# gonewest818/raytrace-clj

Hardware: AMD Instinct MI355X
Metric: Msamples/sec (nx*ny*ns) (higher is better)
Workload: dtype f64; 1 GPU; C3: 1920x1080x256spp Shirley cover scene n=50 (10001 spheres), depth 50, thin-lens camera, seeded counter RNG; accel=bvh; 8x8 tiles dealt round-robin to 1 GPU(s); nx=1920, ny=1080, ns=256, spheres=10001, depth=50, accel=bvh, accel_ran=bvh, frames_in_flight=1, launch_form=one GPU

## Files before the change

include/rtmi.h:

```cpp
#ifndef RTMI_H
#define RTMI_H

#include <stdint.h>

#ifdef __cplusplus
extern "C" {
#endif

#define RTMI_OK 0
#define RTMI_E_ARG (-1)
#define RTMI_E_DEVICE (-2)
#define RTMI_E_UNSUPPORTED (-3)
#define RTMI_E_NOMEM (-4)
#define RTMI_E_STATE (-5)

enum { RTMI_PRIM_SPHERE = 0, RTMI_PRIM_UVSPHERE = 1, RTMI_PRIM_MOVING = 2,
       RTMI_PRIM_RECT_XY = 3, RTMI_PRIM_RECT_XZ = 4, RTMI_PRIM_RECT_YZ = 5, RTMI_PRIM_TRIANGLE = 6,
       RTMI_PRIM_MEDIUM = 7, RTMI_PRIM_BOUNDARY = 16 };
enum { RTMI_XFORM_TRANSLATE = 0, RTMI_XFORM_ROTATE_Y = 1 };
enum { RTMI_MAT_LAMBERTIAN = 0, RTMI_MAT_METAL = 1, RTMI_MAT_DIELECTRIC = 2, RTMI_MAT_DIFFUSE_LIGHT = 3,
       RTMI_MAT_ISOTROPIC = 4  };
enum { RTMI_TEX_CONSTANT = 0, RTMI_TEX_UVGRADIENT = 1, RTMI_TEX_CHECKER = 2,
       RTMI_TEX_PERLIN_NOISE = 3, RTMI_TEX_PERLIN_TURB = 4, RTMI_TEX_MARBLE = 5, RTMI_TEX_FLIP_U = 6, RTMI_TEX_FLIP_V = 7,
       RTMI_TEX_IMAGE = 8 };
// ... 20 lines not shown
int rtmi_shutdown(rtmi_ctx *ctx);
int rtmi_set_option(rtmi_ctx *ctx, const char *name, int64_t value);
int rtmi_device_info(rtmi_ctx *ctx, int32_t *compute_units, int32_t *lds_bytes_per_cu, int64_t *hbm_bytes, char *arch, int32_t arch_len);

int rtmi_scene_create(rtmi_ctx *ctx,
                      int32_t n_prims, const int32_t *prim_kind, const double *prim_geom, const int32_t *prim_mat,
                      int32_t n_mats, const int32_t *mat_kind, const int32_t *mat_tex, const double *mat_param,
                      int32_t n_tex, const int32_t *tex_kind, const double *tex_param, const int32_t *tex_child,
                      int32_t cam_kind, const double *cam, rtmi_scene **out_scene);
int rtmi_scene_create_ex(rtmi_ctx *ctx,
                         int32_t n_prims, const int32_t *prim_kind, const double *prim_geom, const int32_t *prim_mat,
                         int32_t n_mats, const int32_t *mat_kind, const int32_t *mat_tex, const double *mat_param,
                         int32_t n_tex, const int32_t *tex_kind, const double *tex_param, const int32_t *tex_child,
                         int32_t cam_kind, const double *cam,
                         const int32_t *prim_flip, const int32_t *prim_xform,
                         int32_t n_xforms, const int32_t *xform_kind, const double *xform_param, rtmi_scene **out_scene);
int rtmi_scene_set_perlin(rtmi_scene *scene, const double *vectors, const int32_t *perm);
int rtmi_scene_set_images(rtmi_scene *scene, int32_t n_images, const int32_t *wh, const uint8_t *rgb);
int rtmi_scene_set_media_calls(rtmi_scene *scene, int32_t n_calls, const int32_t *calls);
enum { RTMI_MEDIA_DESCENT = 0, RTMI_MEDIA_HITLIST = 1 };
int rtmi_scene_set_media_mode(rtmi_scene *scene, int32_t mode);
int rtmi_scene_set_media_calls_narrowed(rtmi_scene *scene, int32_t n_calls, const int32_t *calls, const int32_t *narrow_from);
int rtmi_scene_device_bytes(rtmi_scene *scene, int64_t *out_bytes);
int rtmi_scene_destroy(rtmi_scene *scene);

int rtmi_render(rtmi_scene *scene, int32_t nx, int32_t ny, int32_t ns, int32_t depth, uint64_t seed, int32_t precision,
                int32_t x0, int32_t y0, int32_t x1, int32_t y1,
                double *out_linear, uint8_t *out_rgb8, uint64_t *out_counters);

int rtmi_render_device(rtmi_scene *scene, int32_t nx, int32_t ny, int32_t ns, int32_t depth, uint64_t seed, int32_t precision,
                       void *d_out_linear, void *d_out_rgb8, void *d_out_counters, void *stream);

int rtmi_render_tiles_device(rtmi_scene *scene, int32_t nx, int32_t ny, int32_t ns, int32_t depth, uint64_t seed, int32_t precision,
                             int32_t tile_first, int32_t tile_stride,
                             void *d_tiles_linear, void *d_out_counters, void *stream);
int32_t rtmi_local_tiles(int32_t nx, int32_t ny, int32_t tile_first, int32_t tile_stride);

int rtmi_render_progressive(rtmi_scene *scene, int32_t nx, int32_t ny, int32_t s_first, int32_t s_count, int32_t depth, uint64_t seed,
                            int32_t precision, int32_t x0, int32_t y0, int32_t x1, int32_t y1,
                            double *out_linear, uint8_t *out_rgb8, double *out_stderr, uint64_t *out_counters);
int rtmi_render_progressive_device(rtmi_scene *scene, int32_t nx, int32_t ny, int32_t s_first, int32_t s_count, int32_t depth, uint64_t seed,
                                   int32_t precision, void *d_out_linear, void *d_out_rgb8, void *d_out_stderr, void *d_out_counters, void *stream);
int rtmi_progressive_samples(rtmi_ctx *ctx, int32_t *samples);
int rtmi_progressive_release(rtmi_ctx *ctx);

int rtmi_assemble_device(rtmi_ctx *ctx, int32_t nx, int32_t ny, int32_t world, int32_t tiles_per_rank,
                         const void *d_gathered, void *d_out_linear, void *d_out_rgb8, void *stream);

int rtmi_scene_clone(rtmi_scene *scene, rtmi_ctx *ctx, rtmi_scene **out_scene);
int rtmi_render_multi(int32_t n, rtmi_scene *const *scenes, int32_t nx, int32_t ny, int32_t ns, int32_t depth, uint64_t seed,
                      int32_t precision, double *out_linear, uint8_t *out_rgb8, uint64_t *out_counters);
int rtmi_render_multi_device(int32_t n, rtmi_scene *const *scenes, int32_t nx, int32_t ny, int32_t ns, int32_t depth, uint64_t seed,
                             int32_t precision, void *d_out_linear, void *d_out_rgb8, void *d_out_counters);
enum { RTMI_GATHER_NONE = 0,
       RTMI_GATHER_SAME_DEVICE = 1,
       RTMI_GATHER_PEER_COPY = 2,
       RTMI_GATHER_RCCL = 3 };
int rtmi_last_gather_path(rtmi_ctx *ctx0, int32_t *path);
int rtmi_rccl_probe(const char *soname);
int rtmi_stream_idle(rtmi_ctx *ctx, int32_t *idle);
int rtmi_last_passes(rtmi_ctx *ctx, int32_t *passes);
int rtmi_last_accel(rtmi_ctx *ctx, int32_t *accel);
int rtmi_last_gather_ms(rtmi_ctx *ctx0, double *ms);

int rtmi_last_traversal_counters(rtmi_ctx *ctx, uint64_t *out_aabb_tests, uint64_t *out_prim_tests);

int rtmi_last_trace_ms(rtmi_ctx *ctx, double *ms, int32_t *launches);
int rtmi_last_reduce_ms(rtmi_ctx *ctx, double *ms, int32_t *launches);

int rtmi_probe_hit(rtmi_scene *scene, int32_t precision, int32_t n, const double *rays, double t_min, double t_max, double *out);
int rtmi_probe_paths(rtmi_scene *scene, int32_t precision, int32_t n, const double *rays, const uint64_t *keys, uint64_t ctr0,
                     int32_t depth, double *out_rgb, uint64_t *out_nseg, double *log, int32_t max_seg, int32_t *out_nlog);
int rtmi_probe_camera(rtmi_scene *scene, int32_t precision, int32_t n, const double *uv, const uint64_t *keys, double *out);
int rtmi_probe_texture(rtmi_scene *scene, int32_t precision, int32_t tex, int32_t n, const double *uvp, double *out);
int rtmi_probe_scatter(rtmi_scene *scene, int32_t precision, int32_t mat, int32_t n, const double *rays, const double *hits,
                       const uint64_t *keys, double *out);
int rtmi_probe_rng(rtmi_ctx *ctx, int32_t precision, uint64_t key, uint64_t d0, int32_t n, uint64_t *out_bits, double *out_real);
uint64_t rtmi_sample_key(uint64_t seed, uint64_t pixel, uint64_t sample);
int rtmi_probe_arith(rtmi_ctx *ctx, int32_t n, const double *abc, double *out);
#define RTMI_PROBE_MATH_SLOTS 12
int rtmi_probe_math2(rtmi_ctx *ctx, int32_t n, const double *abc, double tmin, double tmax, int32_t n_slots, double *out);
int rtmi_probe_math(rtmi_ctx *ctx, int32_t n, const double *abc, double tmin, double tmax, double *out);

int rtmi_test_build_tree(int32_t n, const double *geom, const double *cam, int32_t threads, uint64_t *out_hash, int32_t *out_info, double *out_ms);
int rtmi_test_half_outward(double x, int32_t up);

#ifdef __cplusplus
}
#endif
#endif
```

raytrace_clj_amd/_ffi.py:

```python
import ctypes as C
import os

import numpy as np

try:
    import torch
except ImportError:
    torch = None

_HERE = os.path.dirname(os.path.abspath(__file__))
LIB_PATH = os.environ.get("RTMI_LIB") or os.path.join(_HERE, "lib", "librtmi.so")

SYMBOLS = [
    "rtmi_last_error", "rtmi_backend_name", "rtmi_version", "rtmi_init", "rtmi_shutdown", "rtmi_set_option",
    "rtmi_device_info", "rtmi_scene_create", "rtmi_scene_create_ex", "rtmi_scene_set_perlin", "rtmi_scene_set_images", "rtmi_scene_set_media_calls", "rtmi_scene_set_media_mode", "rtmi_scene_set_media_calls_narrowed", "rtmi_scene_device_bytes", "rtmi_scene_destroy", "rtmi_render", "rtmi_render_device",
    "rtmi_render_tiles_device", "rtmi_local_tiles", "rtmi_assemble_device", "rtmi_last_trace_ms", "rtmi_last_reduce_ms", "rtmi_probe_hit",
    "rtmi_probe_paths", "rtmi_probe_camera", "rtmi_probe_texture", "rtmi_probe_scatter", "rtmi_probe_rng",
    "rtmi_sample_key", "rtmi_test_half_outward", "rtmi_test_build_tree", "rtmi_probe_arith", "rtmi_probe_math", "rtmi_probe_math2", "rtmi_last_traversal_counters",
    "rtmi_scene_clone", "rtmi_render_multi", "rtmi_render_multi_device", "rtmi_last_gather_ms",
    "rtmi_last_gather_path", "rtmi_rccl_probe", "rtmi_stream_idle", "rtmi_last_passes", "rtmi_last_accel",
    "rtmi_render_progressive", "rtmi_render_progressive_device", "rtmi_progressive_samples", "rtmi_progressive_release",
]

F64, F32 = 0, 1
ACCEL_FLAT, ACCEL_BVH = 0, 1
FLAG_TIMING = 1
GATHER_PATHS = {0: "none", 1: "same-device", 2: "peer-copy", 3: "rccl"}
SEG_REC = 12
TILE = 8


class RtmiError(RuntimeError):
    def __init__(self, code, msg):
        super().__init__("rtmi error %d: %s" % (code, msg))
        self.code = code


_lib = None


def lib():
    global _lib
    if _lib is not None:
        return _lib
    if not os.path.exists(LIB_PATH):
        raise RtmiError(-2, "HIP extension %s is missing; build it with `make -C raytrace_clj_amd/csrc` "
                            "(there is no CPU fallback)" % LIB_PATH)
    L = C.CDLL(LIB_PATH)
    vp, i32, i64, u64, dbl = C.c_void_p, C.c_int32, C.c_int64, C.c_uint64, C.c_double
    L.rtmi_last_error.restype = C.c_char_p
    L.rtmi_backend_name.restype = C.c_char_p
    L.rtmi_version.restype = C.c_int
    L.rtmi_init.argtypes = [C.c_int, C.c_uint32, C.POINTER(vp)]
    L.rtmi_shutdown.argtypes = [vp]
    L.rtmi_set_option.argtypes = [vp, C.c_char_p, i64]
    L.rtmi_device_info.argtypes = [vp, C.POINTER(i32), C.POINTER(i32), C.POINTER(i64), C.c_char_p, i32]
    L.rtmi_scene_create.argtypes = [vp, i32, vp, vp, vp, i32, vp, vp, vp, i32, vp, vp, vp, i32, vp, C.POINTER(vp)]
    L.rtmi_scene_create_ex.argtypes = [vp, i32, vp, vp, vp, i32, vp, vp, vp, i32, vp, vp, vp, i32, vp, vp, vp, i32, vp, vp, C.POINTER(vp)]
    L.rtmi_scene_set_perlin.argtypes = [vp, vp, vp]
    L.rtmi_scene_set_images.argtypes = [vp, i32, vp, vp]
    L.rtmi_scene_set_media_calls.argtypes = [vp, i32, vp]
    L.rtmi_scene_set_media_mode.argtypes = [vp, i32]
    L.rtmi_scene_set_media_calls_narrowed.argtypes = [vp, i32, vp, vp]
    L.rtmi_scene_device_bytes.argtypes = [vp, C.POINTER(C.c_int64)]
    L.rtmi_scene_destroy.argtypes = [vp]
    L.rtmi_render.argtypes = [vp, i32, i32, i32, i32, u64, i32, i32, i32, i32, i32, vp, vp, vp]
    L.rtmi_render_device.argtypes = [vp, i32, i32, i32, i32, u64, i32, vp, vp, vp, vp]
    L.rtmi_render_tiles_device.argtypes = [vp, i32, i32, i32, i32, u64, i32, i32, i32, vp, vp, vp]
    L.rtmi_local_tiles.argtypes = [i32, i32, i32, i32]
    L.rtmi_local_tiles.restype = i32
    L.rtmi_assemble_device.argtypes = [vp, i32, i32, i32, i32, vp, vp, vp, vp]
    L.rtmi_last_trace_ms.argtypes = [vp, C.POINTER(dbl), C.POINTER(i32)]
    L.rtmi_last_reduce_ms.argtypes = [vp, C.POINTER(dbl), C.POINTER(i32)]
    L.rtmi_probe_hit.argtypes = [vp, i32, i32, vp, dbl, dbl, vp]
    L.rtmi_probe_paths.argtypes = [vp, i32, i32, vp, vp, u64, i32, vp, vp, vp, i32, vp]
    L.rtmi_probe_camera.argtypes = [vp, i32, i32, vp, vp, vp]
    L.rtmi_probe_texture.argtypes = [vp, i32, i32, i32, vp, vp]
    L.rtmi_probe_scatter.argtypes = [vp, i32, i32, i32, vp, vp, vp, vp]
    L.rtmi_probe_rng.argtypes = [vp, i32, u64, u64, i32, vp, vp]
    L.rtmi_sample_key.argtypes = [u64, u64, u64]
    L.rtmi_sample_key.restype = u64
    L.rtmi_probe_arith.argtypes = [vp, i32, vp, vp]
    L.rtmi_test_build_tree.argtypes = [i32, vp, vp, i32, vp, vp, vp]
    L.rtmi_test_half_outward.argtypes = [C.c_double, i32]
    L.rtmi_probe_math.argtypes = [vp, i32, vp, C.c_double, C.c_double, vp]
    L.rtmi_probe_math2.argtypes = [vp, i32, vp, C.c_double, C.c_double, i32, vp]
    L.rtmi_last_traversal_counters.argtypes = [vp, C.POINTER(u64), C.POINTER(u64)]
    L.rtmi_scene_clone.argtypes = [vp, vp, C.POINTER(vp)]
    L.rtmi_render_multi.argtypes = [i32, C.POINTER(vp), i32, i32, i32, i32, u64, i32, vp, vp, vp]
    L.rtmi_render_multi_device.argtypes = [i32, C.POINTER(vp), i32, i32, i32, i32, u64, i32, vp, vp, vp]
    L.rtmi_last_gather_ms.argtypes = [vp, C.POINTER(dbl)]
    L.rtmi_last_gather_path.argtypes = [vp, C.POINTER(i32)]
    L.rtmi_rccl_probe.argtypes = [C.c_char_p]
    L.rtmi_stream_idle.argtypes = [vp, C.POINTER(i32)]
    L.rtmi_last_passes.argtypes = [vp, C.POINTER(i32)]
    L.rtmi_last_accel.argtypes = [vp, C.POINTER(i32)]
    L.rtmi_render_progressive.argtypes = [vp, i32, i32, i32, i32, i32, u64, i32, i32, i32, i32, i32, vp, vp, vp, vp]
    L.rtmi_render_progressive_device.argtypes = [vp, i32, i32, i32, i32, i32, u64, i32, vp, vp, vp, vp, vp]
    L.rtmi_progressive_samples.argtypes = [vp, C.POINTER(i32)]
    L.rtmi_progressive_release.argtypes = [vp]
    for name in SYMBOLS:
        fn = getattr(L, name)
        if fn.restype is C.c_int and name not in ("rtmi_version",):
            fn.restype = C.c_int
    _lib = L
    return L


def check(rc):
    if rc != 0:
        raise RtmiError(rc, lib().rtmi_last_error().decode("utf-8", "replace"))


def ptr(a):
    if a is None:
        return None
    if isinstance(a, int):
        return C.c_void_p(a)
    if isinstance(a, np.ndarray):
        return a.ctypes.data_as(C.c_void_p)
    if hasattr(a, "data_ptr"):
        return C.c_void_p(a.data_ptr())
    raise TypeError("cannot take a pointer of %r" % type(a))
```

raytrace_clj_amd/core.py:

```python
import ctypes as C
import sys
import time

import numpy as np

from . import _ffi
from . import camera as cam
from . import flatten as fl
from . import hitable as hitm
from . import shader as shad
from . import texture as texm
from ._ffi import F32, F64, RtmiError, check, ptr

T_MIN = 0.001
T_MAX = 3.4028234663852886e38
DEFAULT_DEPTH = 50
RENDER_SEED = 0x5EED0002

_PRECISION = {"f64": F64, "f32": F32, F64: F64, F32: F32}


class Context:

    def __init__(self, device=0, timing=False):
# ... 138 lines not shown
        return lin, q, err, cnt

    def render_progressive_device(self, nx, ny, s_first, s_count, out_linear=None, out_rgb8=None, out_stderr=None, out_counters=None,
                                  depth=DEFAULT_DEPTH, seed=RENDER_SEED, precision="f64", stream=None):
        check(_ffi.lib().rtmi_render_progressive_device(self.handle, nx, ny, s_first, s_count, depth, seed, _PRECISION[precision],
                                                        ptr(out_linear), ptr(out_rgb8), ptr(out_stderr), ptr(out_counters), ptr(stream)))

    def refine(self, nx, ny, ns, chunk, depth=DEFAULT_DEPTH, seed=RENDER_SEED, precision="f64", region=None):
        if chunk <= 0 or ns <= 0:
            raise ValueError("ns and chunk must be > 0")
        k = 0
        while k < ns:
            n = min(chunk, ns - k)
            lin, q, err, cnt = self.render_progressive(nx, ny, k, n, depth, seed, precision, region)
            k += n
            yield k, lin, q, err, cnt

    def render_tiles_device(self, nx, ny, ns, tile_first, tile_stride, out_tiles, out_counters=None, depth=DEFAULT_DEPTH,
                            seed=RENDER_SEED, precision="f64", stream=None):
        check(_ffi.lib().rtmi_render_tiles_device(self.handle, nx, ny, ns, depth, seed, _PRECISION[precision],
                                                  tile_first, tile_stride, ptr(out_tiles), ptr(out_counters), ptr(stream)))

    def probe_hit(self, rays, t_min=T_MIN, t_max=T_MAX, precision="f64"):
        rays = np.ascontiguousarray(rays, np.float64).reshape(-1, 7)
        out = np.zeros((len(rays), 11), np.float64)
        check(_ffi.lib().rtmi_probe_hit(self.handle, _PRECISION[precision], len(rays), ptr(rays), t_min, t_max, ptr(out)))
        return out

    def probe_paths(self, rays, keys, depth=DEFAULT_DEPTH, ctr0=0, max_seg=0, precision="f64"):
        rays = np.ascontiguousarray(rays, np.float64).reshape(-1, 7)
        keys = np.ascontiguousarray(keys, np.uint64)
        n = len(rays)
        rgb, nseg, nlog = np.zeros((n, 3)), np.zeros(n, np.uint64), np.zeros(n, np.int32)
        log = np.zeros((n, max_seg, _ffi.SEG_REC)) if max_seg else None
        check(_ffi.lib().rtmi_probe_paths(self.handle, _PRECISION[precision], n, ptr(rays), ptr(keys), ctr0, depth,
                                          ptr(rgb), ptr(nseg), ptr(log), max_seg, ptr(nlog)))
        return rgb, nseg, log, nlog

    def probe_camera(self, uv, keys, precision="f64"):
        uv = np.ascontiguousarray(uv, np.float64).reshape(-1, 2)
        keys = np.ascontiguousarray(keys, np.uint64)
        out = np.zeros((len(uv), 8))
        check(_ffi.lib().rtmi_probe_camera(self.handle, _PRECISION[precision], len(uv), ptr(uv), ptr(keys), ptr(out)))
        return out

    def probe_texture(self, tex, uvp, precision="f64"):
        uvp = np.ascontiguousarray(uvp, np.float64).reshape(-1, 5)
        out = np.zeros((len(uvp), 3))
        check(_ffi.lib().rtmi_probe_texture(self.handle, _PRECISION[precision], int(tex), len(uvp), ptr(uvp), ptr(out)))
        return out

    def probe_scatter(self, mat, rays, hits, keys, precision="f64"):
        rays = np.ascontiguousarray(rays, np.float64).reshape(-1, 7)
        hits = np.ascontiguousarray(hits, np.float64).reshape(-1, 8)
        keys = np.ascontiguousarray(keys, np.uint64)
        out = np.zeros((len(rays), 9))
        check(_ffi.lib().rtmi_probe_scatter(self.handle, _PRECISION[precision], int(mat), len(rays), ptr(rays), ptr(hits),
                                            ptr(keys), ptr(out)))
        return out


def probe_rng(key, d0, n, precision="f64", ctx=None):
    ctx = ctx or default_context()
    bits, real = np.zeros(n, np.uint64), np.zeros(n, np.float64)
    check(_ffi.lib().rtmi_probe_rng(ctx.handle, _PRECISION[precision], key, d0, n, ptr(bits), ptr(real)))
    return bits, real


def probe_arith(abc, ctx=None):
    ctx = ctx or default_context()
    abc = np.ascontiguousarray(abc, np.float64).reshape(-1, 3)
    out = np.zeros_like(abc)
    check(_ffi.lib().rtmi_probe_arith(ctx.handle, len(abc), ptr(abc), ptr(out)))
    return out


def probe_math(abc, tmin=0.001, tmax=3.4028234663852886e38, ctx=None):
    ctx = ctx or default_context()
    abc = np.ascontiguousarray(abc, np.float64).reshape(-1, 3)
    slots = 12
    out = np.zeros((len(abc), slots))
    check(_ffi.lib().rtmi_probe_math2(ctx.handle, len(abc), ptr(abc), tmin, tmax, slots, ptr(out)))
    return out


def sample_key(seed, pixel, sample):
    return int(_ffi.lib().rtmi_sample_key(seed, pixel, sample))


_dummy_camera = None


def _one_off(world_items, camera=None):
    global _dummy_camera
    if camera is None:
        if _dummy_camera is None:
            _dummy_camera = cam.PinholeCamera(np.zeros(3), np.zeros(3), np.zeros(3), np.zeros(3))
        camera = _dummy_camera
    return DeviceScene(hitm.Hitlist(list(world_items)), camera)


def _ray7(r):
    return np.concatenate([np.asarray(r["origin"], np.float64), np.asarray(r["direction"], np.float64), [float(r["time"])]])


def hit(obj, r, t_min, t_max):
    items = [obj] if not isinstance(obj, (list, tuple)) else obj
    ds = _one_off(items)
    try:
        o = ds.probe_hit(_ray7(r), float(t_min), float(t_max))[0]
        leaves = []
        fl._leaves(items, leaves, set())
    finally:
        ds.close()
    if o[0] == 0:
        return None
    return {"t": o[2], "p": o[3:6].copy(), "uv": (o[9], o[10]), "normal": o[6:9].copy(), "material": leaves[int(o[1])][0].material}


class _Holder(hitm.Sphere):
    pass


def scatter(material, ray_in, hrec, key=0):
    ds = _one_off([hitm.Sphere(np.zeros(3), 1.0, material)])
    try:
        uv = hrec.get("uv", (0.0, 0.0))
        h = np.concatenate([np.asarray(hrec["p"], np.float64), np.asarray(hrec["normal"], np.float64), [uv[0], uv[1]]])
        o = ds.probe_scatter(0, _ray7(ray_in), h, np.array([key], np.uint64))[0]
    finally:
        ds.close()
    if o[0] == 0:
        return None
    return {"scattered": {"origin": np.asarray(hrec["p"], np.float64), "direction": o[1:4].copy(), "time": o[7]},
            "attenuation": o[4:7].copy()}


def emitted(material, uv, p):
    if isinstance(material, shad.DiffuseLight):
        return sample(material.tex, uv, p)
    return np.zeros(3)


def sample(tex, uv, p):
    ds = _one_off([hitm.Sphere(np.zeros(3), 1.0, shad.Lambertian(tex))])
    try:
        t = int(ds.flat.mat_tex[0])
        return ds.probe_texture(t, np.concatenate([[uv[0], uv[1]], np.asarray(p, np.float64)]))[0]
    finally:
        ds.close()


def get_ray(camera, u, v, key=0):
    ds = _one_off([], camera)
    try:
        o = ds.probe_camera(np.array([u, v], np.float64), np.array([key], np.uint64))[0]
    finally:
        ds.close()
    return {"origin": o[0:3].copy(), "direction": o[3:6].copy(), "time": o[6]}


def render(scene, nx, ny, ns, depth=DEFAULT_DEPTH, seed=RENDER_SEED, precision="f64", ctx=None):
    ds = DeviceScene(scene, ctx=ctx)
    try:
        return ds.render(nx, ny, ns, depth, seed, precision)
    finally:
# ... 125 lines not shown
```

raytrace_clj_amd/csrc/rtmi.hip:

```cpp
#include <hip/hip_runtime.h>
#include <rccl/rccl.h>
#include <dlfcn.h>

#include <algorithm>
#include <atomic>
#include <chrono>
#include <condition_variable>
#include <functional>
#include <thread>
#include <cmath>
#include <cmath>
#include <cstdarg>
#include <cstdio>
#include <cstdlib>
#include <cstring>
#include <array>
#include <map>
#include <mutex>
#include <new>
#include <string>
#include <vector>

#include "rtmi.h"
#include "rtmi_device.h"

using namespace rtmi;

#define RTMI_EXPORT extern "C" __attribute__((visibility("default")))

namespace {

constexpr int kBlock = RTMI_TRACE_BLOCK;
constexpr int kTraceBlock = RTMI_TRACE_BLOCK;
#ifdef RTMI_STAMPS
__device__ unsigned long long g_wg_t[2][4096];
__device__ inline unsigned long long real_now() { unsigned long long t; asm volatile("s_memrealtime %0\n\ts_waitcnt lgkmcnt(0)" : "=s"(t)::"memory"); return t; }
#define RTMI_STAMP_DECL const unsigned long long st_wg0 = real_now(); \
    if (lane == 0) for (int k_ = 0; k_ < 3 * PH_SLOTS + 2; ++k_) g_ph[threadIdx.x >> 6][k_] = 0; \
    ph_stamp(-1); for (int k_ = 0; k_ < 32; ++k_) ph_stamp(PH_CAL);
#define RTMI_STAMP_FLUSH(cnt) if (lane == 0) for (int k_ = 0; k_ < 3 * PH_SLOTS; ++k_) if (g_ph[threadIdx.x >> 6][k_]) atomicAdd(&g_phase[k_], g_ph[threadIdx.x >> 6][k_]); \
    __syncthreads(); if (threadIdx.x == 0 && blockIdx.x < 4096) { g_wg_t[0][blockIdx.x] = st_wg0; g_wg_t[1][blockIdx.x] = real_now(); }
#else
#define RTMI_STAMP_DECL
#define RTMI_STAMP_FLUSH(cnt)
#endif
#ifndef RTMI_MIN_WAVES
#define RTMI_MIN_WAVES 4
#endif
#ifndef RTMI_EXT_MIN_WAVES
#define RTMI_EXT_MIN_WAVES RTMI_MIN_WAVES
#endif

struct TraceParams {
    int nx, ny, depth;
    u64 seed;
    int tiles_x;
    int n_local_tiles;
    const int *tile_ids;
    int s_begin, s_count;
    void *samples;
    u64 *counters;
    int prims_per_tile;
    int n_ptiles;
    unsigned *queue;
    unsigned total_items;
    unsigned qblock;
    int suspend_lanes;
    int rx0, ry0, rx1, ry1;
    u64 *trav;
    int susp_off;
    int stash_off;
};
#ifndef RTMI_QUEUE_BLOCK
#define RTMI_QUEUE_BLOCK 256
#endif
#ifndef RTMI_EXT_NO_STASH
#define RTMI_EXT_NO_STASH 0
#endif
#ifndef RTMI_EXT_LDS_STASH
#define RTMI_EXT_LDS_STASH 1
#endif
#ifndef RTMI_STASH
#define RTMI_STASH 1
#endif
constexpr unsigned kQueueBlock = RTMI_QUEUE_BLOCK;

template <typename R> __device__ inline const R *stat4_of(SceneRef sc);
template <typename R> __device__ inline void stage_prims(SceneRef sc, Prim4<R> *lds, int first, int count) {
    for (int i = threadIdx.x; i < count; i += blockDim.x) {
        const R *g = stat4_of<R>(sc) + (size_t)(first + i) * 4;
        Prim4<R> p;
        p.cx = g[0]; p.cy = g[1]; p.cz = g[2]; p.r2 = g[3];
        lds[i] = p;
    }
}

template <typename R> __device__ inline const R *stat4_of(SceneRef sc);
template <> __device__ inline const double *stat4_of<double>(SceneRef sc) { return sc.stat4_d; }
template <> __device__ inline const float *stat4_of<float>(SceneRef sc) { return sc.stat4_f; }

__device__ inline void scan_cull_dispatch(SceneRef sc, const Path<double> &P, double a, double tmin, double &best_t, int &best_i) {
    scan_all_cull(sc, P, a, tmin, best_t, best_i);
}
__device__ inline void scan_cull_dispatch(SceneRef sc, const Path<float> &P, float a, float tmin, float &best_t, int &best_i) {
    scan_static_pipe<float, false>(ScalarPrims<float>(sc.stat4_f), sc.n_static, 0, P, a, tmin, best_t, best_i);
    if (best_i >= 0) best_i = sc.stat_orig[best_i];
    if (sc.n_moving > 0) {
        int best_orig = best_i >= 0 ? best_i : 0x7fffffff, scan_i = -1;
        scan_moving<float>(sc, P, a, tmin, best_t, scan_i, best_orig);
        if (scan_i >= 0) best_i = best_orig;
    }
}


template <bool SLICED = false, bool COUNT = false, int MSEQ = 0>
__device__ inline void intersect_ext(SceneRef sc, int *stack, bool bvh, Path<double> &P, bool active, double tmin, double tmax, double &best_t, int &best_i,
                                     bool *mid = nullptr, int min_lanes = 0, unsigned *cnt = nullptr, int susp_off = RTMI_BVH_STACK * RTMI_BVH_STRIDE) {
    best_t = tmax; best_i = -1;
    if (!active) return;
    const double a = dot3(P.dx, P.dy, P.dz, P.dx, P.dy, P.dz);
    ExtHit H = {tmax, 0x7fffffff, -1};
    if (MSEQ == 2) {
        MediumChord chord = medium_chord_begin(P);
        ExtHit Hrun = {tmax, 0x7fffffff, -1};
        int cur_lo = -1, scanned_to = 0;
        for (int k = 0; k < sc.n_media; ++k) {
            const int m = sc.media_idx[k], lo = sc.media_lo[k];
            if (lo >= m) { ext_medium_test(sc, m, P, tmin, tmax, H, chord, COUNT ? cnt : nullptr); continue; }
            if (lo != cur_lo) { Hrun.t = tmax; Hrun.F = 0x7fffffff; Hrun.W = -1; cur_lo = lo; scanned_to = lo; }
            if (m > scanned_to) scan_all_cull_ext(sc, P, a, tmin, Hrun, scanned_to, m);
            double tm = 0.0;
            if (ext_medium_test(sc, m, P, tmin, Hrun.any() ? Hrun.t : tmax, Hrun, chord, COUNT ? cnt : nullptr, &tm)) ext_update(H, tm, m, true);
            scanned_to = m + 1;
        }
        if (bvh) scan_bvh_ext<false, COUNT>(sc, stack, P, a, tmin, H, nullptr, false, 0, cnt);
        else if (sc.small_scan) scan_small_ext(sc, P, tmin, H);
        else scan_all_cull_ext(sc, P, a, tmin, H);
        best_i = ext_winner(H);
        if (best_i >= 0) best_t = H.t;
        return;
    }
    if (MSEQ == 1) {
        int prev = 0;
        MediumChord chord = medium_chord_begin(P);
        for (int k = 0; k <= sc.n_media; ++k) {
            const int m = k < sc.n_media ? sc.media_idx[k] : sc.n_all;
            if (m > prev) {
                if (bvh) scan_bvh_ext<false, COUNT>(sc, stack, P, a, tmin, H, nullptr, false, 0, cnt, prev, m);
                else if (sc.small_scan) scan_small_ext(sc, P, tmin, H, prev, m);
                else scan_all_cull_ext(sc, P, a, tmin, H, prev, m);
            }
            if (k < sc.n_media) ext_medium_test(sc, m, P, tmin, H.any() ? H.t : tmax, H, chord, COUNT ? cnt : nullptr);
            prev = m + 1;
        }
        best_i = ext_winner(H);
        if (best_i >= 0) best_t = H.t;
        return;
    }
    if (!(SLICED && bvh && *mid)) {
        MediumChord chord = medium_chord_begin(P);
        for (int k = 0; k < sc.n_media; ++k) ext_medium_test(sc, sc.media_idx[k], P, tmin, tmax, H, chord, COUNT ? cnt : nullptr, nullptr, k);
        RTMI_PH(PH_MEDIA)
    }
    if (bvh) {
        if (SLICED) {
            const bool done = scan_bvh_ext<true, COUNT>(sc, stack, P, a, tmin, H, stack + susp_off, *mid, min_lanes, cnt);
            *mid = !done;
            if (!done) return;
        } else scan_bvh_ext<false, COUNT>(sc, stack, P, a, tmin, H, nullptr, false, 0, cnt);
    } else if (sc.small_scan) scan_small_ext(sc, P, tmin, H);
    else scan_all_cull_ext(sc, P, a, tmin, H);
    RTMI_PH(PH_BVH_POST)
    best_i = ext_winner(H);
    if (best_i >= 0) best_t = H.t;
}
template <bool SLICED = false, bool COUNT = false, int MSEQ = 0>
__device__ inline void intersect_ext(SceneRef, int *, bool, Path<float> &, bool, float, float tmax, float &best_t, int &best_i, bool * = nullptr, int = 0, unsigned * = nullptr, int = 0) { best_t = tmax; best_i = -1; }

template <typename R, bool MULTI, int VARIANT, bool EXT = false, bool COUNT = false, bool SLICED = false, int MSEQ = 0, bool NOGRID = false>
__device__ inline void intersect_world(SceneRef sc, Prim4<R> *lds, int prims_per_tile, int n_ptiles, Path<R> &P,
                                       bool active, R tmin, R tmax, R &best_t, int &best_i, unsigned *cnt = nullptr, bool *mid = nullptr, int min_lanes = 0,
                                       int susp_off = RTMI_BVH_STACK * RTMI_BVH_STRIDE) {
    if (EXT) { intersect_ext<SLICED, COUNT, MSEQ>(sc, reinterpret_cast<int *>(lds), VARIANT == SCAN_BVH, P, active, tmin, tmax, best_t, best_i, mid, min_lanes, cnt, susp_off); return; }
    best_t = tmax;
    best_i = -1;
    const R a = dot3(P.dx, P.dy, P.dz, P.dx, P.dy, P.dz);
    if (VARIANT == SCAN_BVH) {
        int *stack = reinterpret_cast<int *>(lds);
        if (active) {
            if (SLICED) {
                const bool done = scan_bvh<R, COUNT, true>(sc, stack, P, a, tmin, best_t, best_i, [&]() { scan_cull_dispatch(sc, P, a, tmin, best_t, best_i); }, cnt,
                                                           stack + susp_off, *mid, min_lanes);
                *mid = !done;
            } else scan_bvh<R, COUNT, false, !NOGRID>(sc, stack, P, a, tmin, best_t, best_i, [&]() { scan_cull_dispatch(sc, P, a, tmin, best_t, best_i); }, cnt);
        }
        return;
    }
    if (VARIANT == SCAN_SGPR_CULL) {
        if (active) scan_cull_dispatch(sc, P, a, tmin, best_t, best_i);
        return;
    }
    if (VARIANT == SCAN_SGPR) {
        if (active) scan_static_pipe<R, false>(ScalarPrims<R>(stat4_of<R>(sc)), sc.n_static, 0, P, a, tmin, best_t, best_i);
    } else if (!MULTI) {
        if (active) {
            if (VARIANT == SCAN_LDS_PIPE) scan_static_pipe<R, true>(LdsPrims<R>{lds}, sc.n_static, 0, P, a, tmin, best_t, best_i);
            else scan_static<R>(lds, sc.n_static, 0, P, a, tmin, best_t, best_i);
        }
    } else {
        for (int tile = 0; tile < n_ptiles; ++tile) {
            const int first = tile * prims_per_tile;
            const int count = min(prims_per_tile, sc.n_static - first);
            __syncthreads();
            stage_prims<R>(sc, lds, first, count);
            __syncthreads();
            if (active) {
                if (VARIANT == SCAN_LDS_PIPE) scan_static_pipe<R, true>(LdsPrims<R>{lds}, count, first, P, a, tmin, best_t, best_i);
                else scan_static<R>(lds, count, first, P, a, tmin, best_t, best_i);
            }
        }
    }
    if (active) {
        if (best_i >= 0) best_i = sc.stat_orig[best_i];
        if (sc.n_moving > 0) {
            int best_orig = best_i >= 0 ? best_i : 0x7fffffff, scan_i = -1;
            scan_moving<R>(sc, P, a, tmin, best_t, scan_i, best_orig);
            if (scan_i >= 0) best_i = best_orig;
        }
    }
}

template <typename R> __device__ inline void start_sample(SceneRef sc, const TraceParams &tp, int i, int j, int s, Path<R> &P) {
    seed_stream(P, sample_key(tp.seed, (u64)j * (u64)tp.nx + (u64)i, (u64)s), 0u);
    const R u = ((R)(float)i + next_uniform(P)) / (R)tp.nx;
    const R v = ((R)(float)j + next_uniform(P)) / (R)tp.ny;
    get_ray<R>(sc, u, v, P);
    P.ar = P.ag = P.ab = R(1);
    P.depth = tp.depth;
}

template <typename R, bool MULTI, int VARIANT, bool EXT = false, bool COUNT = false, bool SLICE = true, int MSEQ = 0, bool LST = false>
__global__ void __launch_bounds__(kTraceBlock, EXT ? ((MSEQ != 0 || COUNT) ? 3 : RTMI_EXT_MIN_WAVES) : RTMI_MIN_WAVES) trace_kernel(ScenePtr scp, TraceParams tp) {
    SceneRef sc = *scp;
    extern __shared__ __attribute__((aligned(16))) char smem[];
    Prim4<R> *lds = reinterpret_cast<Prim4<R> *>(smem);
    const int lane = threadIdx.x & 63;
    if (!MULTI && VARIANT < SCAN_SGPR) stage_prims<R>(sc, lds, 0, sc.n_static);
    __syncthreads();

    const unsigned total_items = tp.total_items;
    unsigned w_cur = 0, w_end = 0;
    Path<R> P;
    P.ox = P.oy = P.oz = P.dx = P.dy = P.dz = P.time = R(0);
    P.ar = P.ag = P.ab = R(0);
    seed_stream(P, 0ull, 0u); P.depth = 0;
    bool alive = false;
    bool exhausted = (total_items == 0);
    unsigned out_item = 0;
    constexpr bool LSTASH = (EXT && RTMI_STASH && RTMI_EXT_LDS_STASH && !RTMI_EXT_NO_STASH) || LST;
    constexpr bool STASH = RTMI_STASH && !(EXT && RTMI_EXT_NO_STASH) && !LSTASH;
    int *const lst = reinterpret_cast<int *>(smem) + tp.stash_off + (threadIdx.x & ~63);
    R st_ox = R(0), st_oy = R(0), st_oz = R(0), st_dx = R(0), st_dy = R(0), st_dz = R(0), st_time = R(0);
    u64 st_rs = 0;
    unsigned st_item = 0xffffffffu;
    unsigned s_head = 64u;
    unsigned nrays = 0;
    unsigned ntrav[2] = {0u, 0u};
    const R tmin = R(0.001), tmax = Real<R>::tmax();
    constexpr bool SLICED = SLICE && VARIANT == SCAN_BVH && !MULTI;
    bool mid = false;

    RTMI_STAMP_DECL
    for (;;) {
        RTMI_PH(PH_LOOP)
        if (LSTASH) {
        for (;;) {
            const u64 dead = __ballot(!alive);
            if (dead == 0) break;
            if (s_head == 64u) {
                if (exhausted) break;
                if (w_cur == w_end) {
                    unsigned base = 0;
                    if (lane == 0) base = atomicAdd(tp.queue, tp.qblock);
                    base = __builtin_amdgcn_readfirstlane(base);
                    if (base >= total_items) { exhausted = true; break; }
                    w_cur = base;
                    w_end = min(base + tp.qblock, total_items);
                }
                const unsigned m = w_cur + (unsigned)lane;
                w_cur += 64u;
                const unsigned chunk = m >> 6;
                const int l = (int)(m & 63u);
                const int tile_local = (int)(chunk / (unsigned)tp.s_count);
                const int s = tp.s_begin + (int)(chunk - (unsigned)tile_local * (unsigned)tp.s_count);
                const int gtile = tp.tile_ids[tile_local];
                const int x = (gtile % tp.tiles_x) * RTMI_TILE + (l & 7);
                const int y = (gtile / tp.tiles_x) * RTMI_TILE + (l >> 3);
                unsigned item = 0xffffffffu;
                if (x >= tp.rx0 && x < tp.rx1 && y >= tp.ry0 && y < tp.ry1) {
                    Path<R> Q;
                    start_sample<R>(sc, tp, x, tp.ny - 1 - y, s, Q);
                    int w0, w1;
                    best_to_words<R>(Q.dx, w0, w1); lst[lane] = w0; lst[kTraceBlock + lane] = w1;
                    best_to_words<R>(Q.dy, w0, w1); lst[2 * kTraceBlock + lane] = w0; lst[3 * kTraceBlock + lane] = w1;
                    best_to_words<R>(Q.dz, w0, w1); lst[4 * kTraceBlock + lane] = w0; lst[5 * kTraceBlock + lane] = w1;
                    best_to_words<R>(Q.time, w0, w1); lst[6 * kTraceBlock + lane] = w0; lst[7 * kTraceBlock + lane] = w1;
                    lst[8 * kTraceBlock + lane] = (int)(unsigned)Q.rs; lst[9 * kTraceBlock + lane] = (int)(unsigned)(Q.rs >> 32);
                    if (!sc.cam_fixed_origin) {
                        best_to_words<R>(Q.ox, w0, w1); lst[11 * kTraceBlock + lane] = w0; lst[12 * kTraceBlock + lane] = w1;
                        best_to_words<R>(Q.oy, w0, w1); lst[13 * kTraceBlock + lane] = w0; lst[14 * kTraceBlock + lane] = w1;
                        best_to_words<R>(Q.oz, w0, w1); lst[15 * kTraceBlock + lane] = w0; lst[16 * kTraceBlock + lane] = w1;
                    }
                    item = m;
                    RTMI_PH(PH_REFILL_GEN)
                }
                lst[10 * kTraceBlock + lane] = (int)item;
                s_head = 0u;
            }
// ... 713 lines not shown
    fprintf(stderr, "[phases] one stamp = %.0f ticks; stamps took %.1f %% of the %.4g wave-ticks of this (diagnostic) launch and are subtracted below\n", per_stamp, 100 * (raw - tot) / raw, raw);
    fprintf(stderr, "[phases] %-36s %8s %8s %10s %10s %12s\n", "phase", "ticks %", "lanes", "masked %", "useful %", "stamps");
    for (int k = 0; k < PH_N; ++k) {
        if (!h[k] || k == PH_CAL) continue;
        const double t = tk[k], l = lk[k];
        fprintf(stderr, "[phases] %-36s %8.2f %8.1f %10.2f %10.2f %12llu\n", names[k], 100 * t / tot, t > 0 ? l / t : 0.0, 100 * (64 * t - l) / (64 * tot), 100 * l / (64 * tot), h[2 * PH_SLOTS + k]);
    }
    fprintf(stderr, "[phases] %-36s %8.2f %8.1f %10.2f %10.2f   (%.4g wave-ticks)\n", "total", 100.0, totl / tot, 100 * (64 * tot - totl) / (64 * tot), 100 * totl / (64 * tot), tot);
    return RTMI_OK;
}
#endif

template <typename R>
int render_passes(rtmi_scene *s, int nx, int ny, int s_first, int s_end, int depth, uint64_t seed, int first, int stride, const int *rg, void *d_tiles_linear,
                  void *d_counters, hipStream_t st, ProgFrame *prog) {
    rtmi_ctx *c = s->ctx;
    int n_local = 0;
    const int whole[4] = {0, 0, nx, ny};
    if (!rg) rg = whole;
    int rc = ensure_tile_ids(c, nx, ny, first, stride, rg, st, &n_local);
    if (rc) return rc;
    c->last_stream = st;
    if (c->fail_next_render) { c->fail_next_render = 0; return fail(RTMI_E_DEVICE, "render failed (injected by the test hook test_fail_next_render)"); }
    if (prog) {
        prog->k = 0;
        const size_t elems = (size_t)std::max(n_local, 1) * 192;
        if (s_first == 0) {
            rc = prog->sums.ensure(elems * sizeof(R));
            if (!rc) rc = prog->mean.ensure(elems * sizeof(double));
            if (!rc) rc = prog->m2.ensure(elems * sizeof(double));
            if (!rc) rc = prog->counters.ensure(2 * sizeof(u64));
            if (rc) return rc;
            HIP_TRY(hipMemsetAsync(prog->counters.p, 0, 2 * sizeof(u64), st));
        } else if (prog->sums.bytes < elems * sizeof(R) || prog->m2.bytes < elems * sizeof(double)) {
            return fail(RTMI_E_STATE, "progressive frame buffers do not match the frame");
        }
        d_counters = prog->counters.p;
    }
    rc = c->counters.ensure(8 * sizeof(u64));
    if (rc) return rc;
    if (d_counters && !prog) HIP_TRY(hipMemsetAsync(d_counters, 0, 2 * sizeof(u64), st));
    HIP_TRY(hipMemsetAsync(reinterpret_cast<u64 *>(c->counters.p) + 3, 0, 2 * sizeof(u64), st));
    if (n_local == 0) return RTMI_OK;
    u64 *cnt = d_counters ? reinterpret_cast<u64 *>(d_counters) : reinterpret_cast<u64 *>(c->counters.p);
    unsigned *queue = reinterpret_cast<unsigned *>(reinterpret_cast<u64 *>(c->counters.p) + 2);

    const int ns = s_end - s_first;
    const size_t per_sample = (size_t)n_local * 64 * 3 * sizeof(R);
    int s_per_pass = (int)std::max<int64_t>(1, std::min<int64_t>(ns, c->workspace_bytes / (int64_t)per_sample));
    while (s_per_pass > 1 && (long long)n_local * s_per_pass * 64 >= 0xf0000000ll) s_per_pass /= 2;
    if ((long long)n_local * s_per_pass * 64 >= 0xf0000000ll) return fail(RTMI_E_ARG, "frame too large for one pass: %d tiles per rank", n_local);
    if (per_sample * (size_t)s_per_pass > c->samples.bytes) {
        constexpr double kFreeShare = 0.8;
        size_t free_b = 0, total_b = 0;
        if (hipMemGetInfo(&free_b, &total_b) == hipSuccess) {
            const double avail = kFreeShare * (double)free_b + (double)c->samples.bytes;
            const int fit = (int)std::max<double>(1.0, std::min<double>((double)s_per_pass, avail / (double)per_sample));
            s_per_pass = std::min(s_per_pass, fit);
        }
        for (;;) {
            if (c->fail_allocs > 0) { c->fail_allocs--; c->samples.release(); rc = fail(RTMI_E_NOMEM, "hipMalloc(%zu bytes) failed (injected by the test hook)", per_sample * (size_t)s_per_pass); }
            else rc = c->samples.ensure(per_sample * (size_t)s_per_pass);
            if (!rc) break;
            (void)hipGetLastError();
            if (s_per_pass == 1) return rc;
            s_per_pass = (s_per_pass + 1) / 2;
        }
    }
    c->last_passes = (ns + s_per_pass - 1) / s_per_pass;
    if (!prog && s_per_pass < ns) {
        rc = c->accum.ensure((size_t)n_local * 64 * 3 * sizeof(R));
        if (rc) return rc;
    }
    int ppt, nptiles;
    size_t lds_bytes;
    lds_plan(c, s->dev.n_static, sizeof(R), &ppt, &nptiles, &lds_bytes);
    const TracePlan plan = choose_trace_kernel<R>(s, c, read_launch_knobs(), nptiles > 1, lds_bytes);
    c->last_accel = plan.accel;

    for (int s_begin = s_first; s_begin < s_end; s_begin += s_per_pass) {
        const int s_count = std::min(s_per_pass, s_end - s_begin);
        TraceParams tp;
        tp.nx = nx; tp.ny = ny; tp.depth = depth; tp.seed = seed; tp.tiles_x = tiles_x_of(nx);
        tp.n_local_tiles = n_local; tp.tile_ids = reinterpret_cast<const int *>(c->tile_ids.p);
        tp.s_begin = s_begin; tp.s_count = s_count; tp.samples = c->samples.p; tp.counters = cnt;
        tp.prims_per_tile = (c->scan_variant >= SCAN_SGPR || s->dev.has_ext) ? 0 : ppt; tp.n_ptiles = nptiles;
        hipEvent_t e0 = nullptr, e1 = nullptr;
        if ((c->flags & RTMI_FLAG_TIMING) && c->events_used < 8192) {
            rc = next_event_pair(c, &e0, &e1);
            if (rc) return rc;
            HIP_TRY(hipEventRecord(e0, st));
        }
        tp.queue = queue; tp.total_items = (unsigned)((long long)n_local * s_count * 64);
        {
            const long long per_wave = (long long)tp.total_items / std::max(1, c->cus * 16);
            unsigned qb = s->dev.has_ext ? 192u : kQueueBlock;
            while (qb < 1024u && per_wave >= (long long)qb * 128) qb *= 2;
            if (const char *e = std::getenv("RTMI_QUEUE_BLOCK_RT")) qb = std::max(64, std::atoi(e) / 64 * 64);
            tp.qblock = qb;
        }
        tp.rx0 = std::max(rg[0], 0); tp.ry0 = std::max(rg[1], 0); tp.rx1 = std::min(rg[2], nx); tp.ry1 = std::min(rg[3], ny);
        tp.trav = reinterpret_cast<u64 *>(c->counters.p) + 3;
        tp.suspend_lanes = plan.suspend_lanes; tp.susp_off = plan.lds.susp_off; tp.stash_off = plan.lds.stash_off;
        HIP_TRY(hipMemsetAsync(queue, 0, sizeof(unsigned), st));
        int resident = 0;
        {
            const std::pair<const void *, size_t> key(reinterpret_cast<const void *>(plan.kern), plan.lds.bytes);
            auto it = c->occupancy.find(key);
            if (it == c->occupancy.end()) {
                HIP_TRY(hipOccupancyMaxActiveBlocksPerMultiprocessor(&resident, plan.kern, kTraceBlock, plan.lds.bytes));
                c->occupancy.emplace(key, resident);
            } else resident = it->second;
        }
        const int grid_trace = std::max(1, c->cus * std::max(1, std::min(c->blocks_per_cu * (256 / kTraceBlock), resident)));
        if (c->last_grid != grid_trace && std::getenv("RTMI_DEBUG"))
            fprintf(stderr, "[rtmi] trace launch: %d workgroups of %d threads (%d resident per CU by the occupancy query, cap %d), %zu B LDS each\n",
                    grid_trace, kTraceBlock, resident, c->blocks_per_cu * (256 / kTraceBlock), plan.lds.bytes);
        c->last_grid = grid_trace;
        hipLaunchKernelGGL(plan.kern, dim3(grid_trace), dim3(kTraceBlock), plan.lds.bytes, st, s->d_dev, tp);
        HIP_TRY(hipGetLastError());
        if (e1) HIP_TRY(hipEventRecord(e1, st));
        const long long npx = (long long)n_local * 64;
        if (prog)
            hipLaunchKernelGGL((progressive_fold_kernel<R>), dim3((unsigned)((npx + kBlock - 1) / kBlock)), dim3(kBlock), 0, st,
                               reinterpret_cast<const R *>(c->samples.p), reinterpret_cast<R *>(prog->sums.p), reinterpret_cast<double *>(prog->mean.p),
                               reinterpret_cast<double *>(prog->m2.p), reinterpret_cast<const int *>(c->tile_ids.p), tiles_x_of(nx), n_local,
                               s_begin, s_count, cnt, (u64)c->tile_valid_pixels, tp.rx0, tp.ry0, tp.rx1, tp.ry1);
        else
            hipLaunchKernelGGL((reduce_kernel<R>), dim3((unsigned)((npx + kBlock - 1) / kBlock)), dim3(kBlock), 0, st,
                               reinterpret_cast<const R *>(c->samples.p), reinterpret_cast<R *>(c->accum.p),
                               reinterpret_cast<double *>(d_tiles_linear), reinterpret_cast<const int *>(c->tile_ids.p), tiles_x_of(nx), nx, ny,
                               n_local, s_begin, s_count, ns, d_counters ? cnt : nullptr, (u64)c->tile_valid_pixels, tp.rx0, tp.ry0, tp.rx1, tp.ry1);
        HIP_TRY(hipGetLastError());
        if (e1) {
            const size_t k = (size_t)c->events_used - 1;
            while (c->events_r.size() <= k) { hipEvent_t e; HIP_TRY(hipEventCreate(&e)); c->events_r.push_back(e); }
            HIP_TRY(hipEventRecord(c->events_r[k], st));
        }
    }
#ifdef RTMI_STAMPS
    rc = report_phase_stamps(c, st);
#endif
    if (!rc && prog) prog->k = s_end;
    return rc;
}

template <typename R>
int render_tiles_impl(rtmi_scene *s, int nx, int ny, int ns, int depth, uint64_t seed, int first, int stride, const int *rg, void *d_tiles_linear,
                      void *d_counters, hipStream_t st) {
    return render_passes<R>(s, nx, ny, 0, ns, depth, seed, first, stride, rg, d_tiles_linear, d_counters, st, nullptr);
}

int check_render_args(rtmi_scene *s, int nx, int ny, int ns, int depth, int precision) {
    if (!scene_ok(s)) return fail(RTMI_E_STATE, "invalid scene handle");
    if (nx <= 0 || ny <= 0 || ns <= 0 || depth < 0) return fail(RTMI_E_ARG, "nx, ny, ns must be > 0 and depth >= 0 (got %d %d %d %d)", nx, ny, ns, depth);
    if ((long long)nx * ny > (1ll << 30)) return fail(RTMI_E_ARG, "frame too large");
    if (precision != RTMI_F64 && precision != RTMI_F32) return fail(RTMI_E_ARG, "precision must be RTMI_F64 or RTMI_F32");
    if (precision == RTMI_F32 && s->dev.has_ext) return fail(RTMI_E_UNSUPPORTED, "rectangles / triangles / instances / procedural textures are rendered by the FP64 kernels only");
    if (s->uses_perlin && !s->have_perlin) return fail(RTMI_E_STATE, "the scene holds a Perlin texture: call rtmi_scene_set_perlin first");
    if (s->max_image >= s->dev.n_images) return fail(RTMI_E_STATE, "the scene holds an ImageMap with index %d: call rtmi_scene_set_images first", s->max_image);
    return RTMI_OK;
}

}

RTMI_EXPORT int rtmi_test_build_tree(int32_t n, const double *geom, const double *cam, int32_t threads, uint64_t *out_hash, int32_t *out_info, double *out_ms) {
    if (n <= 0 || !geom || !cam || !out_hash || !out_info || !out_ms) return fail(RTMI_E_ARG, "bad arguments");
    const BuildKnobs knobs = read_build_knobs();
    std::vector<int> kind((size_t)n, RTMI_PRIM_SPHERE);
    std::vector<BvhBox> wbox((size_t)n);
    std::vector<char> bounded((size_t)n, 0), box_first((size_t)n, 0);
    for (int i = 0; i < n; ++i) {
        const double g[9] = {geom[4 * (size_t)i], geom[4 * (size_t)i + 1], geom[4 * (size_t)i + 2], geom[4 * (size_t)i + 3], 0, 0, 0, 0, 1};
        bounded[(size_t)i] = prim_world_box(RTMI_PRIM_SPHERE, g, nullptr, nullptr, 0, 0, 0.0, 1.0, wbox[(size_t)i]);
    }
    DevScene d{};
    std::vector<int> grid_cells;
    int depth = 0;
    g_build_single.store(threads == 1 ? 1 : 0);
    const double t0 = now_ms();
    const std::vector<float> nodes = build_bvh(d, n, kind.data(), wbox, bounded, cam, true, grid_cells, box_first, knobs, &depth);
    *out_ms = now_ms() - t0;
    g_build_single.store(0);
    uint64_t h = 1469598103934665603ull;
    auto mix = [&](const void *p, size_t bytes) { const unsigned char *q = (const unsigned char *)p; for (size_t k = 0; k < bytes; ++k) { h ^= q[k]; h *= 1099511628211ull; } };
    mix(nodes.data(), nodes.size() * sizeof(float));
    mix(grid_cells.data(), grid_cells.size() * sizeof(int));
    mix(&d.bvh_root, sizeof(int)); mix(&d.grid_tall, sizeof(int)); mix(&d.bvh_node16, sizeof(int));
    *out_hash = h;
    out_info[0] = (int32_t)(nodes.size() / (d.bvh_node16 ? 8 : 16)); out_info[1] = depth; out_info[2] = d.grid_n; out_info[3] = d.n_big;
    return RTMI_OK;
}
RTMI_EXPORT int rtmi_test_half_outward(double x, int32_t up) { return (int)half_outward((float)x, up != 0); }
RTMI_EXPORT const char *rtmi_last_error(void) { return g_err.c_str(); }
RTMI_EXPORT const char *rtmi_backend_name(void) { return "hip-gfx950"; }
RTMI_EXPORT int rtmi_version(void) { return 205; }
RTMI_EXPORT uint64_t rtmi_sample_key(uint64_t seed, uint64_t pixel, uint64_t sample) { return sample_key(seed, pixel, sample); }

RTMI_EXPORT int rtmi_init(int device, uint32_t flags, rtmi_ctx **out_ctx) {
    if (!out_ctx) return fail(RTMI_E_ARG, "out_ctx is NULL");
    *out_ctx = nullptr;
    int ndev = 0;
    if (hipGetDeviceCount(&ndev) != hipSuccess || ndev <= 0) return fail(RTMI_E_DEVICE, "no HIP device visible (this library has no CPU fallback)");
    if (device < 0 || device >= ndev) return fail(RTMI_E_ARG, "device %d out of range (0..%d)", device, ndev - 1);
    HIP_TRY(hipSetDevice(device));
    hipDeviceProp_t prop;
    HIP_TRY(hipGetDeviceProperties(&prop, device));
    if (std::strncmp(prop.gcnArchName, "gfx950", 6) != 0)
        return fail(RTMI_E_DEVICE, "device %d is %s; this library carries gfx950 (MI355X) code objects only", device, prop.gcnArchName);
    rtmi_ctx *c = new (std::nothrow) rtmi_ctx();
    if (!c) return fail(RTMI_E_NOMEM, "out of host memory");
    c->device = device;
    c->flags = flags;
    c->cus = prop.multiProcessorCount;
    c->lds_per_cu = (int)prop.maxSharedMemoryPerMultiProcessor;
    c->hbm = prop.totalGlobalMem;
    c->arch = prop.gcnArchName;
    if (const char *e = std::getenv("RTMI_BLOCKS_PER_CU")) c->blocks_per_cu = std::max(1, std::atoi(e));
    if (const char *e = std::getenv("RTMI_SCAN_VARIANT")) c->scan_variant = std::min(3, std::max(0, std::atoi(e)));
    if (const char *e = std::getenv("RTMI_LDS_TILE_BYTES")) c->max_lds_bytes = std::min(64 * 1024 - 64, std::max(1024, std::atoi(e)));
    if (hipStreamCreateWithFlags(&c->stream, hipStreamNonBlocking) != hipSuccess) { delete c; return fail(RTMI_E_DEVICE, "hipStreamCreate failed"); }
    *out_ctx = c;
    return RTMI_OK;
}

RTMI_EXPORT int rtmi_shutdown(rtmi_ctx *c) {
    if (!ctx_ok(c)) return fail(RTMI_E_STATE, "invalid context handle");
    (void)hipSetDevice(c->device);
    (void)hipStreamSynchronize(c->stream);
#ifdef RTMI_HIST
    { unsigned long long h[200]; if (hipMemcpyFromSymbol(h, HIP_SYMBOL(rtmi::g_hist), sizeof h) == hipSuccess) { for (int k = 0; k < 3; ++k) { fprintf(stderr, "HIST%d", k); for (int i = 0; i <= 64; ++i) fprintf(stderr, " %llu", h[64 * k + i]); fprintf(stderr, "\n"); } } }
#endif
    c->samples.release(); c->accum.release(); c->tiles.release(); c->tile_ids.release(); c->counters.release(); c->scratch_lin.release(); c->multi.release();
    c->prog.release();
    for (hipEvent_t e : {c->ev_done, c->ev_g0, c->ev_g1}) if (e) (void)hipEventDestroy(e);
    if (c->ev_consumed) { (void)hipSetDevice(c->ev_consumed_device); (void)hipEventDestroy(c->ev_consumed); (void)hipSetDevice(c->device); }
    for (auto &e : c->events) { (void)hipEventDestroy(e.first); (void)hipEventDestroy(e.second); }
    for (hipEvent_t e : c->events_r) (void)hipEventDestroy(e);
    (void)hipStreamDestroy(c->stream);
    c->magic = 0;
    delete c;
    return RTMI_OK;
}

RTMI_EXPORT int rtmi_set_option(rtmi_ctx *c, const char *name, int64_t value) {
    if (!ctx_ok(c)) return fail(RTMI_E_STATE, "invalid context handle");
    if (!name) return fail(RTMI_E_ARG, "name is NULL");
    if (!std::strcmp(name, "blocks_per_cu")) { if (value < 1 || value > 64) return fail(RTMI_E_ARG, "blocks_per_cu must be 1..64"); c->blocks_per_cu = (int)value; return RTMI_OK; }
    if (!std::strcmp(name, "workspace_bytes")) { if (value < (1 << 20)) return fail(RTMI_E_ARG, "workspace_bytes must be >= 1 MiB"); c->workspace_bytes = value; return RTMI_OK; }
    if (!std::strcmp(name, "lds_tile_bytes")) { if (value < 1024 || value > 64 * 1024 - 64) return fail(RTMI_E_ARG, "lds_tile_bytes out of range"); c->max_lds_bytes = (int)value; return RTMI_OK; }
    if (!std::strcmp(name, "timing")) { if (value) c->flags |= RTMI_FLAG_TIMING; else c->flags &= ~RTMI_FLAG_TIMING; return RTMI_OK; }
    if (!std::strcmp(name, "scan_variant")) { if (value < 0 || value > 3) return fail(RTMI_E_ARG, "scan_variant must be 0..3"); c->scan_variant = (int)value; return RTMI_OK; }
    if (!std::strcmp(name, "count_traversal")) { c->count_traversal = value ? 1 : 0; return RTMI_OK; }
    if (!std::strcmp(name, "test_fail_next_render")) { c->fail_next_render = value ? 1 : 0; return RTMI_OK; }
    if (!std::strcmp(name, "test_fail_allocs")) { c->fail_allocs = (int)std::max<int64_t>(0, std::min<int64_t>(value, 64)); return RTMI_OK; }
    if (!std::strcmp(name, "flat_below")) { if (value < 0 || value > (1 << 20)) return fail(RTMI_E_ARG, "flat_below must be 0..2^20"); c->flat_below = (int)value; return RTMI_OK; }
    if (!std::strcmp(name, "suspend_lanes")) { if (value < 0 || value > 64) return fail(RTMI_E_ARG, "suspend_lanes must be 0..64"); c->suspend_lanes = (int)value; c->suspend_lanes_set = true; return RTMI_OK; }
    if (!std::strcmp(name, "accel")) {
        if (value == RTMI_ACCEL_FLAT || value == RTMI_ACCEL_BVH) { c->accel = (int)value; return RTMI_OK; }
        return fail(RTMI_E_UNSUPPORTED, "accel %lld is not available in this build", (long long)value);
    }
    return fail(RTMI_E_ARG, "unknown option '%s'", name);
}

RTMI_EXPORT int rtmi_device_info(rtmi_ctx *c, int32_t *cus, int32_t *lds, int64_t *hbm, char *arch, int32_t arch_len) {
    if (!ctx_ok(c)) return fail(RTMI_E_STATE, "invalid context handle");
    if (cus) *cus = c->cus;
    if (lds) *lds = c->lds_per_cu;
    if (hbm) *hbm = (int64_t)c->hbm;
    if (arch && arch_len > 0) { std::strncpy(arch, c->arch.c_str(), (size_t)arch_len - 1); arch[arch_len - 1] = 0; }
    return RTMI_OK;
}

RTMI_EXPORT int rtmi_scene_create(rtmi_ctx *c, int32_t n_prims, const int32_t *prim_kind, const double *prim_geom, const int32_t *prim_mat,
                                  int32_t n_mats, const int32_t *mat_kind, const int32_t *mat_tex, const double *mat_param,
                                  int32_t n_tex, const int32_t *tex_kind, const double *tex_param, const int32_t *tex_child,
                                  int32_t cam_kind, const double *cam, rtmi_scene **out_scene) {
    return rtmi_scene_create_ex(c, n_prims, prim_kind, prim_geom, prim_mat, n_mats, mat_kind, mat_tex, mat_param, n_tex, tex_kind, tex_param, tex_child,
                                cam_kind, cam, nullptr, nullptr, 0, nullptr, nullptr, out_scene);
// ... 886 lines not shown
    else hipLaunchKernelGGL((probe_camera_kernel<float>), dim3(grid), dim3(kBlock), 0, c->stream, s->d_dev, n, d_uv, d_keys, d_out);
    PROBE_EPILOGUE()
    HIP_TRY(hipMemcpy(out, d_out, (size_t)n * 8 * sizeof(double), hipMemcpyDeviceToHost));
    return RTMI_OK;
}

RTMI_EXPORT int rtmi_probe_texture(rtmi_scene *s, int32_t precision, int32_t tex, int32_t n, const double *uvp, double *out) {
    PROBE_PROLOGUE(s)
    if (!uvp || !out) return fail(RTMI_E_ARG, "NULL array");
    if (tex < 0 || tex >= s->n_tex) return fail(RTMI_E_ARG, "texture index %d out of range", tex);
    double *d_in = (double *)tmp.up(uvp, (size_t)n * 5 * sizeof(double));
    double *d_out = (double *)tmp.alloc((size_t)n * 3 * sizeof(double));
    if (!d_in || !d_out) return fail(RTMI_E_NOMEM, "probe buffers");
    if (s->dev.has_ext) {
        if (precision != RTMI_F64) return fail(RTMI_E_UNSUPPORTED, "procedural / image textures are FP64 only");
        hipLaunchKernelGGL((probe_texture_kernel<double, true>), dim3(grid), dim3(kBlock), 0, c->stream, s->d_dev, tex, n, d_in, d_out);
    } else if (precision == RTMI_F64) hipLaunchKernelGGL((probe_texture_kernel<double>), dim3(grid), dim3(kBlock), 0, c->stream, s->d_dev, tex, n, d_in, d_out);
    else hipLaunchKernelGGL((probe_texture_kernel<float>), dim3(grid), dim3(kBlock), 0, c->stream, s->d_dev, tex, n, d_in, d_out);
    PROBE_EPILOGUE()
    HIP_TRY(hipMemcpy(out, d_out, (size_t)n * 3 * sizeof(double), hipMemcpyDeviceToHost));
    return RTMI_OK;
}

RTMI_EXPORT int rtmi_probe_scatter(rtmi_scene *s, int32_t precision, int32_t mat, int32_t n, const double *rays, const double *hits,
                                   const uint64_t *keys, double *out) {
    PROBE_PROLOGUE(s)
    if (!rays || !hits || !keys || !out) return fail(RTMI_E_ARG, "NULL array");
    if (mat < 0 || mat >= s->n_mats) return fail(RTMI_E_ARG, "material index %d out of range", mat);
    double *d_rays = (double *)tmp.up(rays, (size_t)n * 7 * sizeof(double));
    double *d_hits = (double *)tmp.up(hits, (size_t)n * 8 * sizeof(double));
    u64 *d_keys = (u64 *)tmp.up(keys, (size_t)n * sizeof(u64));
    double *d_out = (double *)tmp.alloc((size_t)n * 9 * sizeof(double));
    if (!d_rays || !d_hits || !d_keys || !d_out) return fail(RTMI_E_NOMEM, "probe buffers");
    if (s->dev.has_ext) {
        if (precision != RTMI_F64) return fail(RTMI_E_UNSUPPORTED, "procedural / image textures are FP64 only");
        hipLaunchKernelGGL((probe_scatter_kernel<double, true>), dim3(grid), dim3(kBlock), 0, c->stream, s->d_dev, mat, n, d_rays, d_hits, d_keys, d_out);
    } else if (precision == RTMI_F64) hipLaunchKernelGGL((probe_scatter_kernel<double>), dim3(grid), dim3(kBlock), 0, c->stream, s->d_dev, mat, n, d_rays, d_hits, d_keys, d_out);
    else hipLaunchKernelGGL((probe_scatter_kernel<float>), dim3(grid), dim3(kBlock), 0, c->stream, s->d_dev, mat, n, d_rays, d_hits, d_keys, d_out);
    PROBE_EPILOGUE()
    HIP_TRY(hipMemcpy(out, d_out, (size_t)n * 9 * sizeof(double), hipMemcpyDeviceToHost));
    return RTMI_OK;
}

RTMI_EXPORT int rtmi_probe_rng(rtmi_ctx *c, int32_t precision, uint64_t key, uint64_t d0, int32_t n, uint64_t *out_bits, double *out_real) {
    if (!ctx_ok(c)) return fail(RTMI_E_STATE, "invalid context handle");
    if (precision != RTMI_F64 && precision != RTMI_F32) return fail(RTMI_E_ARG, "bad precision");
    if (n <= 0 || !out_bits || !out_real) return fail(RTMI_E_ARG, "bad arguments");
    HIP_TRY(hipSetDevice(c->device));
    Tmp tmp;
    u64 *d_bits = (u64 *)tmp.alloc((size_t)n * sizeof(u64));
    double *d_real = (double *)tmp.alloc((size_t)n * sizeof(double));
    if (!d_bits || !d_real) return fail(RTMI_E_NOMEM, "probe buffers");
    const unsigned grid = (unsigned)((n + kBlock - 1) / kBlock);
    if (precision == RTMI_F64) hipLaunchKernelGGL((probe_rng_kernel<double>), dim3(grid), dim3(kBlock), 0, c->stream, (u64)key, (u64)d0, n, d_bits, d_real);
    else hipLaunchKernelGGL((probe_rng_kernel<float>), dim3(grid), dim3(kBlock), 0, c->stream, (u64)key, (u64)d0, n, d_bits, d_real);
    PROBE_EPILOGUE()
    HIP_TRY(hipMemcpy(out_bits, d_bits, (size_t)n * sizeof(u64), hipMemcpyDeviceToHost));
    HIP_TRY(hipMemcpy(out_real, d_real, (size_t)n * sizeof(double), hipMemcpyDeviceToHost));
    return RTMI_OK;
}

__global__ void probe_math_kernel(int n, const double *abc, double tmin, double tmax, int n_slots, double *out) {
    const int k = blockIdx.x * blockDim.x + threadIdx.x;
    if (k >= n) return;
    const double a = abc[3 * k], b = abc[3 * k + 1], c = abc[3 * k + 2];
    double o[RTMI_PROBE_MATH_SLOTS];
    o[0] = rt_sqrt(a);
    const TrigTable K = trig_table();
    o[1] = rt_atan2(a, b, K);
    o[2] = rt_asin(a, K);
    Real<double>::sphere_uv(a, b, c, &o[3], &o[4]);
    const Quot<double> q = make_quot<double>(b, tmin, tmax);
    o[5] = q(a);
    o[6] = div_const(a, K[29], K[27]);
    o[7] = (double)q.fast;
    o[8] = (double)float_above(c);
    o[9] = rt_log_unit(a);
    const bool fast = rcp_in_range(b) && tmin >= 0x1p-300 && tmax <= 0x1p200;
    o[10] = div_by(a, refined_rcp(b), fast);
    o[11] = (double)fast;
    for (int j = 0; j < n_slots; ++j) out[(size_t)k * n_slots + j] = o[j];
}

RTMI_EXPORT int rtmi_probe_arith(rtmi_ctx *c, int32_t n, const double *abc, double *out) {
    if (!ctx_ok(c)) return fail(RTMI_E_STATE, "invalid context handle");
    if (n <= 0 || !abc || !out) return fail(RTMI_E_ARG, "bad arguments");
    HIP_TRY(hipSetDevice(c->device));
    Tmp tmp;
    double *d_in = (double *)tmp.up(abc, (size_t)n * 3 * sizeof(double));
    double *d_out = (double *)tmp.alloc((size_t)n * 3 * sizeof(double));
    if (!d_in || !d_out) return fail(RTMI_E_NOMEM, "probe buffers");
    const unsigned grid = (unsigned)((n + kBlock - 1) / kBlock);
    hipLaunchKernelGGL(probe_arith_kernel, dim3(grid), dim3(kBlock), 0, c->stream, n, d_in, d_out);
    PROBE_EPILOGUE()
    HIP_TRY(hipMemcpy(out, d_out, (size_t)n * 3 * sizeof(double), hipMemcpyDeviceToHost));
    return RTMI_OK;
}

RTMI_EXPORT int rtmi_probe_math2(rtmi_ctx *c, int32_t n, const double *abc, double tmin, double tmax, int32_t n_slots, double *out) {
    if (!ctx_ok(c)) return fail(RTMI_E_STATE, "invalid context handle");
    if (n <= 0 || !abc || !out) return fail(RTMI_E_ARG, "bad arguments");
    if (n_slots < 1 || n_slots > RTMI_PROBE_MATH_SLOTS) return fail(RTMI_E_ARG, "n_slots must be 1..%d", RTMI_PROBE_MATH_SLOTS);
    HIP_TRY(hipSetDevice(c->device));
    Tmp tmp;
    double *d_in = (double *)tmp.up(abc, (size_t)n * 3 * sizeof(double));
    double *d_out = (double *)tmp.alloc((size_t)n * (size_t)n_slots * sizeof(double));
    if (!d_in || !d_out) return fail(RTMI_E_NOMEM, "probe buffers");
    const unsigned grid = (unsigned)((n + kBlock - 1) / kBlock);
    hipLaunchKernelGGL(probe_math_kernel, dim3(grid), dim3(kBlock), 0, c->stream, n, d_in, tmin, tmax, (int)n_slots, d_out);
    PROBE_EPILOGUE()
    HIP_TRY(hipMemcpy(out, d_out, (size_t)n * (size_t)n_slots * sizeof(double), hipMemcpyDeviceToHost));
    return RTMI_OK;
}
RTMI_EXPORT int rtmi_probe_math(rtmi_ctx *c, int32_t n, const double *abc, double tmin, double tmax, double *out) {
    return rtmi_probe_math2(c, n, abc, tmin, tmax, 8, out);
}
```

raytrace_clj_amd/csrc/rtmi_device.h:

```cpp
#pragma once
#include <hip/hip_runtime.h>
#include <stdint.h>

#include "rtmi.h"

namespace rtmi {

typedef unsigned long long u64;

struct DevScene {
    int n_static;
    int n_moving;
    const double *stat_geom;
    const double *stat4_d;
    const float *stat4_f;
    int n_all;
    const float *cull20;
    const double *exact12;
    double cull_t_lo, cull_t_hi;
    const float *bvh_nodes;
    int bvh_root;
    int n_big;
    int big_idx[16];
    int bvh_node16;
// ... 131 lines not shown
__device__ inline double rt_atan2(double y, double x, TrigTable K) {
    double c_hi = K[11], c_lo = K[12], h_hi = K[13], h_lo = K[14], p_hi = K[15], p_lo = K[16];
    asm volatile("" : "+s"(c_hi), "+s"(c_lo), "+s"(h_hi), "+s"(h_lo), "+s"(p_hi), "+s"(p_lo));
    const double ax = ::fabs(x), ay = ::fabs(y);
    const bool swap = ay > ax;
    const double a = swap ? ax : ay, b = swap ? ay : ax;
    const bool far = a > 0.4375 * b;
    const bool zero = b == 0.0;
    double num = far ? ::fma(-0.75, b, a) : a, den = far ? ::fma(0.75, a, b) : b;
    den = zero ? 1.0 : den;
    const double xr = num / den, z = xr * xr, w = z * z;
    const double s1 = z * fma_s(w, fma_s(w, fma_s(w, fma_s(w, ::fma(w, K[10], K[8]), K[6]), K[4]), K[2]), K[0]);
    const double s2 = w * fma_s(w, fma_s(w, fma_s(w, ::fma(w, K[9], K[7]), K[5]), K[3]), K[1]);
    const double hi = far ? c_hi : 0.0, lo = far ? c_lo : 0.0;
    double r = hi - (::fma(xr, s1 + s2, -lo) - xr);
    const double rs = h_hi - (r - h_lo);
    r = swap ? rs : r;
    const bool neg = (x < 0.0) | (zero & (bool)__builtin_signbit(x));
    const double rn = p_hi - (r - p_lo);
    r = neg ? rn : r;
    return ::copysign(r, y);
}
__device__ inline double rt_asin(double x, TrigTable K) {
    const double ax = ::fabs(x);
    const bool small = ax < 0.5;
    const double t = small ? x * x : ::fma(ax, -0.5, 0.5);
    const double p = t * fma_s(t, fma_s(t, fma_s(t, fma_s(t, ::fma(t, K[22], K[21]), K[20]), K[19]), K[18]), K[17]);
    const double q = ::fma(t, fma_s(t, fma_s(t, ::fma(t, K[26], K[25]), K[24]), K[23]), 1.0);
    const double r = p / q, s = rt_sqrt(t);
    const double big = K[13] - ::fma(2.0, ::fma(s, r, s), -K[14]);
    return ::copysign(small ? ::fma(ax, r, ax) : big, x);
}
__device__ inline double rt_log_unit(double x) {
    const double ln2_hi = 6.93147180369123816490e-01, ln2_lo = 1.90821492927058770002e-10;
    const double Lg1 = 6.666666666666735130e-01, Lg2 = 3.999999999940941908e-01, Lg3 = 2.857142874366239149e-01, Lg4 = 2.222219843214978396e-01,
                 Lg5 = 1.818357216161805012e-01, Lg6 = 1.531383769920937332e-01, Lg7 = 1.479819860511658591e-01;
    int hx = __double2hiint(x);
    const unsigned lx = (unsigned)__double2loint(x);
    if (!(x > 0.0) || hx >= 0x7ff00000) return x == 0.0 ? -__builtin_inf() : ::log(x);
    if (hx < 0x00100000) return ::log(x);
    int k = (hx >> 20) - 1023;
    hx &= 0x000fffff;
    const int i = (hx + 0x95f64) & 0x100000;
    const double m = __hiloint2double(hx | (i ^ 0x3ff00000), (int)lx);
    k += i >> 20;
    const double f = m - 1.0, dk = (double)k;
    const double s = f / (2.0 + f);
    const double z = s * s, w = z * z;
    const double t1 = w * ::fma(w, ::fma(w, Lg6, Lg4), Lg2);
    const double t2 = z * ::fma(w, ::fma(w, ::fma(w, Lg7, Lg5), Lg3), Lg1);
    const double R = t2 + t1, hfsq = 0.5 * f * f;
    return ::fma(dk, ln2_hi, -((hfsq - ::fma(s, hfsq + R, dk * ln2_lo)) - f));
}

__device__ inline double div_const(double x, double c, double rc) {
    const double q = x * rc;
    return ::fma(::fma(-c, q, x), rc, q);
}

template <typename R> struct Quot {
    R a;
    __device__ inline R operator()(R n) const { return n / a; }
};
template <> struct Quot<double> {
    double a, r;
    bool fast;
    __device__ inline double operator()(double n) const {
        if (__builtin_expect(!fast, 0)) return n / a;
        const double q = n * r;
        return ::fma(::fma(-a, q, n), r, q);
    }
};
template <typename R> __device__ inline Quot<R> make_quot(R a, R, R) { return Quot<R>{a}; }
template <> __device__ inline Quot<double> make_quot<double>(double a, double tmin, double tmax) {
    Quot<double> q;
    q.a = a;
    const unsigned hi = (unsigned)__double2hiint(a);
    q.fast = (hi - (823u << 20) < (400u << 20)) && tmin >= 0x1p-300 && tmax <= 0x1p200;
    double r = __builtin_amdgcn_rcp(a);
    r = ::fma(r, ::fma(-a, r, 1.0), r);
    q.r = ::fma(r, ::fma(-a, r, 1.0), r);
    return q;
}
template <typename R> __device__ inline R quot(R n, R a) { return n / a; }
template <typename R> __device__ inline R quot(R n, const Quot<R> &a) { return a(n); }
template <typename R> __device__ inline R coef(R a) { return a; }
template <typename R> __device__ inline R coef(const Quot<R> &a) { return a.a; }

#ifdef RTMI_HIST
__device__ unsigned long long g_hist[200];
#endif
template <typename R> struct Real;
template <> struct Real<double> {
    __device__ static inline double k53(u64 z) { const u64 k = z >> 11; return ::fma((double)(unsigned)(k >> 32), 4294967296.0, (double)(unsigned)k); }
#ifndef RTMI_RNG_BITS
#define RTMI_RNG_BITS 1
#endif
#if RTMI_RNG_BITS
    __device__ static inline double from_bits(u64 z, unsigned expo, unsigned sub_b1, unsigned sub_b0) {
        const unsigned hi = (unsigned)(z >> 32), lo = (unsigned)z;
        const double m = __hiloint2double((int)(expo | ((hi >> 11) & 0x000fffffu)), (int)__builtin_amdgcn_alignbit(hi, lo, 11));
        return m - __hiloint2double((int)hi < 0 ? (int)sub_b1 : (int)sub_b0, 0);
    }
    __device__ static inline double uniform(u64 z) { return from_bits(z, 0x3fe00000u, 0u, 0x3fe00000u); }
    __device__ static inline double symmetric(u64 z) { return from_bits(z, 0x3ff00000u, 0x3ff00000u, 0x40000000u); }
#else
    __device__ static inline double uniform(u64 z) { return k53(z) * (1.0 / 9007199254740992.0); }
    __device__ static inline double symmetric(u64 z) { return ::fma(k53(z), 1.0 / 4503599627370496.0, -1.0); }
#endif
    __device__ static inline double tmax() { return 3.4028234663852886e38; }
    __device__ static inline double pi() { return 3.141592653589793; }
    __device__ static inline double sqrt_(double x) { return rt_sqrt(x); }
    __device__ static inline double sqrt_lib(double x) { return ::sqrt(x); }
    __device__ static inline double sin_(double x) { return ::sin(x); }
    __device__ static inline void sphere_uv(double nx, double ny, double nz, double *u, double *v) { *u = sphere_u(nx, nz); *v = sphere_v(ny); }
    __device__ static inline double sphere_u(double nx, double nz) { const TrigTable K = trig_table(); return 1.0 - div_const(rt_atan2(nz, nx, K) + K[30], K[29], K[27]); }
    __device__ static inline double sphere_v(double ny) { const TrigTable K = trig_table(); return div_const(rt_asin(ny, K) + K[13], K[30], K[28]); }
    __device__ static inline double pow_(double x, double y) { return ::pow(x, y); }
};
template <> struct Real<float> {
    __device__ static inline float uniform(u64 z) { return (float)(unsigned)(z >> 40) * (1.0f / 16777216.0f); }
    __device__ static inline float symmetric(u64 z) { return 2.0f * uniform(z) - 1.0f; }
    __device__ static inline float tmax() { return 3.4028234663852886e38f; }
    __device__ static inline float pi() { return 3.141592653589793f; }
    __device__ static inline float sqrt_(float x) { return ::sqrtf(x); }
    __device__ static inline float sqrt_lib(float x) { return ::sqrtf(x); }
    __device__ static inline float sin_(float x) { return ::sinf(x); }
    __device__ static inline void sphere_uv(float nx, float ny, float nz, float *u, float *v) { *u = sphere_u(nx, nz); *v = sphere_v(ny); }
    __device__ static inline float sphere_u(float nx, float nz) { return 1.0f - (::atan2f(nz, nx) + pi()) / (2.0f * pi()); }
    __device__ static inline float sphere_v(float ny) { return (::asinf(ny) + pi() / 2.0f) / pi(); }
    __device__ static inline float pow_(float x, float y) { return ::powf(x, y); }
};

__device__ inline double pow5(double x) {
    const double h2 = x * x, l2 = ::fma(x, x, -h2);
    const double h4 = h2 * h2, l4 = ::fma(h2, h2, -h4) + 2.0 * (h2 * l2);
    const double h5 = h4 * x, l5 = ::fma(h4, x, -h5) + l4 * x;
    return h5 + l5;
}
__device__ inline float pow5(float x) { const double d = (double)x, d2 = d * d; return (float)(d2 * d2 * d); }

template <typename R> struct Path {
    R ox, oy, oz, dx, dy, dz, time;
    R ar, ag, ab;
    u64 key;
    u64 rs;
    unsigned ctr;
    int depth;
};
template <typename R> __device__ inline void seed_stream(Path<R> &P, u64 key, unsigned ctr0) { P.key = key; P.ctr = ctr0; P.rs = key + RTMI_GOLD * (u64)ctr0; }

template <typename R> __device__ inline R next_uniform(Path<R> &P) {
    P.rs += RTMI_GOLD;
    P.ctr++;
    return Real<R>::uniform(mix64(P.rs));
}

template <typename R> __device__ inline R next_symmetric(Path<R> &P) {
    P.rs += RTMI_GOLD;
    P.ctr++;
    return Real<R>::symmetric(mix64(P.rs));
}

template <typename R> __device__ inline R dot3(R ax, R ay, R az, R bx, R by, R bz) { return (ax * bx + ay * by) + az * bz; }

template <typename R> __device__ inline void rand_in_unit_sphere(Path<R> &P, R &x, R &y, R &z) {
// ... 205 lines not shown
        if (kind == RTMI_TEX_UVGRADIENT) {
            const R omu = R(1.0) - u, omv = R(1.0) - v;
            const R a0 = (R)tp[3] * omu + (R)tp[0] * u, a1 = (R)tp[4] * omu + (R)tp[1] * u, a2 = (R)tp[5] * omu + (R)tp[2] * u;
            const R b0 = (R)tp[9] * omu + (R)tp[6] * u, b1 = (R)tp[10] * omu + (R)tp[7] * u, b2 = (R)tp[11] * omu + (R)tp[8] * u;
            r = b0 * omv + a0 * v; g = b1 * omv + a1 * v; b = b2 * omv + a2 * v;
            return;
        }
        if (kind == RTMI_TEX_CHECKER) {
            const R scale = (R)tp[0];
            const int sx = sin_sign<R>(scale * px), sy = sin_sign<R>(scale * py), sz = sin_sign<R>(scale * pz);
            t = (sx * sy * sz < 0) ? sc.tex_child[2 * t] : sc.tex_child[2 * t + 1];
            continue;
        }
        if (F4) {
            if (kind == RTMI_TEX_PERLIN_NOISE) {
                const R s = (R)tp[0];
                r = g = b = R(0.5) * (perlin_noise<R>(sc, s * px, s * py, s * pz) + R(1.0));
                return;
            }
            if (kind == RTMI_TEX_PERLIN_TURB) {
                const R s = (R)tp[0];
                r = g = b = R(0.5) * (perlin_turbulence<R>(sc, s * px, s * py, s * pz, (int)tp[1]) + R(1.0));
                return;
            }
            if (kind == RTMI_TEX_MARBLE) {
                r = g = b = R(0.5) * (Real<R>::sin_((R)tp[0] * pz + R(10.0) * perlin_turbulence<R>(sc, px, py, pz, (int)tp[1])) + R(1.0));
                return;
            }
            if (kind == RTMI_TEX_FLIP_U) { u = R(1.0) - u; t = sc.tex_child[2 * t]; continue; }
            if (kind == RTMI_TEX_FLIP_V) { v = R(1.0) - v; t = sc.tex_child[2 * t]; continue; }
            if (kind == RTMI_TEX_IMAGE) {
                const int im = (int)tp[0];
                const int w = sc.image_wh[2 * im], h = sc.image_wh[2 * im + 1];
                int i = (int)(u * (R)w), j = (int)(v * (R)h);
                i = i < 0 ? 0 : (i >= w ? w - 1 : i); j = j < 0 ? 0 : (j >= h ? h - 1 : j);
                const unsigned char *q = sc.image_rgb + sc.image_off[im] + ((size_t)j * w + i) * 3;
                r = (R)q[0] / R(255.0); g = (R)q[1] / R(255.0); b = (R)q[2] / R(255.0);
                return;
            }
        }
        return;
    }
}

template <typename R> struct alignas(16) Prim4 { R cx, cy, cz, r2; };

enum { SCAN_LDS_LITERAL = 0, SCAN_LDS_PIPE = 1, SCAN_SGPR = 2, SCAN_SGPR_CULL = 3, SCAN_BVH = 4 };

template <typename R>
__device__ inline void scan_static(const Prim4<R> *__restrict__ lds, int n, int idx_base, const Path<R> &P, R a, R tmin, R &best_t, int &best_i) {
    const R a2 = R(2.0) * a, a4 = R(4.0) * a;
#pragma unroll 2
    for (int i = 0; i < n; ++i) {
        const Prim4<R> s = lds[i];
        const R ocx = P.ox - s.cx, ocy = P.oy - s.cy, ocz = P.oz - s.cz;
        const R b = R(2.0) * dot3(ocx, ocy, ocz, P.dx, P.dy, P.dz);
        const R c = dot3(ocx, ocy, ocz, ocx, ocy, ocz) - s.r2;
        const R disc = b * b - a4 * c;
        if (disc >= R(0)) {
            const R sq = Real<R>::sqrt_lib(disc);
            R t = (-b - sq) / a2;
            bool ok = (t > tmin) && (t < best_t);
            if (!ok) {
                t = (-b + sq) / a2;
                ok = (t > tmin) && (t < best_t);
            }
            if (ok) { best_t = t; best_i = idx_base + i; }
        }
    }
}

template <typename R, typename A>
__device__ inline void sphere_roots(R bq, R cq, R disc, const A &a, R tmin, bool behind_ok, R &best_t, int &best_i, int idx) {
    if (behind_ok && bq > R(0) && cq > R(0)) return;
    const R sq = Real<R>::sqrt_(disc);
    R t = quot<R>(-bq - sq, a);
    bool ok = (t > tmin) && (t < best_t);
    if (!ok) {
        t = quot<R>(-bq + sq, a);
        ok = (t > tmin) && (t < best_t);
    }
    if (ok) { best_t = t; best_i = idx; }
}

template <typename R> __device__ inline void sphere_test(const Prim4<R> &s, const Path<R> &P, R a, R &bq, R &cq, R &disc) {
    const R ocx = P.ox - s.cx, ocy = P.oy - s.cy, ocz = P.oz - s.cz;
    bq = dot3(ocx, ocy, ocz, P.dx, P.dy, P.dz);
    cq = dot3(ocx, ocy, ocz, ocx, ocy, ocz) - s.r2;
    disc = bq * bq - a * cq;
}

template <typename R> struct LdsPrims {
    const Prim4<R> *p;
    __device__ inline Prim4<R> operator()(int i) const { return p[i]; }
};
template <typename R> struct ScalarPrims {
    typedef R v4 __attribute__((ext_vector_type(4)));
    typedef const __attribute__((address_space(4))) v4 *cptr;
    cptr p;
    __device__ explicit ScalarPrims(const R *g) : p((cptr)(g)) {}
    __device__ inline Prim4<R> operator()(int i) const {
        const v4 v = p[i];
        Prim4<R> s; s.cx = v.x; s.cy = v.y; s.cz = v.z; s.r2 = v.w;
        return s;
    }
};

template <typename R> struct Group4 { Prim4<R> s0, s1, s2, s3; };

template <typename R, bool CLAMP, typename Src> __device__ inline Group4<R> load_group(const Src &src, int g, int last) {
    Group4<R> G;
    G.s0 = src(CLAMP ? min(g, last) : g);
    G.s1 = src(CLAMP ? min(g + 1, last) : g + 1);
    G.s2 = src(CLAMP ? min(g + 2, last) : g + 2);
    G.s3 = src(CLAMP ? min(g + 3, last) : g + 3);
    return G;
}

template <typename R>
__device__ inline void test_group(const Group4<R> &G, int g, int last, int idx_base, const Path<R> &P, R a, R tmin, bool behind_ok, R &best_t, int &best_i) {
    R b0, q0, d0, b1, q1, d1, b2, q2, d2, b3, q3, d3;
    sphere_test(G.s0, P, a, b0, q0, d0);
    sphere_test(G.s1, P, a, b1, q1, d1);
    sphere_test(G.s2, P, a, b2, q2, d2);
    sphere_test(G.s3, P, a, b3, q3, d3);
    if ((d0 >= R(0)) | (d1 >= R(0)) | (d2 >= R(0)) | (d3 >= R(0))) {
        if (d0 >= R(0)) sphere_roots(b0, q0, d0, a, tmin, behind_ok, best_t, best_i, idx_base + min(g, last));
        if (d1 >= R(0)) sphere_roots(b1, q1, d1, a, tmin, behind_ok, best_t, best_i, idx_base + min(g + 1, last));
        if (d2 >= R(0)) sphere_roots(b2, q2, d2, a, tmin, behind_ok, best_t, best_i, idx_base + min(g + 2, last));
        if (d3 >= R(0)) sphere_roots(b3, q3, d3, a, tmin, behind_ok, best_t, best_i, idx_base + min(g + 3, last));
    }
}

template <typename R, bool CLAMP, typename Src>
__device__ inline void scan_static_pipe(const Src &src, int n, int idx_base, const Path<R> &P, R a, R tmin, R &best_t, int &best_i) {
    if (n <= 0) return;
    const int last = n - 1;
    const bool behind_ok = tmin >= R(0);
    Group4<R> A = load_group<R, CLAMP>(src, 0, last);
    for (int g = 0; g < n; g += 8) {
        const Group4<R> B = load_group<R, CLAMP>(src, g + 4, last);
        test_group<R>(A, g, last, idx_base, P, a, tmin, behind_ok, best_t, best_i);
        A = load_group<R, CLAMP>(src, g + 8, last);
        test_group<R>(B, g + 4, last, idx_base, P, a, tmin, behind_ok, best_t, best_i);
    }
}

struct CullRay { float ox, oy, oz, dx, dy, dz, a, A0, A1; };

__device__ inline CullRay make_cull_ray(const Path<double> &P, double a, double t_lo, double t_hi) {
    CullRay c;
    c.ox = (float)P.ox; c.oy = (float)P.oy; c.oz = (float)P.oz;
    c.dx = (float)P.dx; c.dy = (float)P.dy; c.dz = (float)P.dz;
    c.a = fmaf(c.dz, c.dz, fmaf(c.dy, c.dy, c.dx * c.dx));
    const float on = (fabsf(c.ox) + fabsf(c.oy)) + fabsf(c.oz);
    const float ku = 64.0f * 5.9604645e-08f;
    c.A1 = ku * c.a * 1.0001f;
    c.A0 = c.A1 * (2.0f * on * on);
    const bool safe = (on < 1e15f) && (c.a > 1e-30f) && (c.a < 1e30f) && (a > 1e-30) && (a < 1e30) && (P.time >= t_lo) && (P.time <= t_hi);
    if (!safe) {
        c.ox = c.oy = c.oz = c.dx = c.dy = c.dz = 0.0f; c.a = 0.0f; c.A1 = 0.0f; c.A0 = 3.0e38f;
    }
    return c;
}

struct CullGroup { float cx[4], cy[4], cz[4], r2[4], w[4]; };

__device__ inline CullGroup load_cull_group(const float *base, int group) {
    typedef float f4 __attribute__((ext_vector_type(4)));
    typedef const __attribute__((address_space(4))) f4 *cptr;
    const cptr p = (cptr)(base) + (size_t)group * 5;
    const f4 x = p[0], y = p[1], z = p[2], r = p[3], w = p[4];
    CullGroup G;
    G.cx[0] = x.x; G.cx[1] = x.y; G.cx[2] = x.z; G.cx[3] = x.w;
    G.cy[0] = y.x; G.cy[1] = y.y; G.cy[2] = y.z; G.cy[3] = y.w;
    G.cz[0] = z.x; G.cz[1] = z.y; G.cz[2] = z.z; G.cz[3] = z.w;
    G.r2[0] = r.x; G.r2[1] = r.y; G.r2[2] = r.z; G.r2[3] = r.w;
    G.w[0] = w.x; G.w[1] = w.y; G.w[2] = w.z; G.w[3] = w.w;
    return G;
}

__device__ inline float cull_disc(const CullGroup &G, int k, const CullRay &c) {
    const float ocx = c.ox - G.cx[k], ocy = c.oy - G.cy[k], ocz = c.oz - G.cz[k];
    const float b = fmaf(ocz, c.dz, fmaf(ocy, c.dy, ocx * c.dx));
    const float q = fmaf(ocz, ocz, fmaf(ocy, ocy, fmaf(ocx, ocx, -G.r2[k])));
    const float t1 = fmaf(c.A1, G.w[k], c.A0);
    const float t2 = fmaf(-c.a, q, t1);
    return fmaf(b, b, t2);
}

template <typename R, typename A>
__device__ inline void exact_prim_test(const double *exact12, int i, int idx, const Path<R> &P, const A &a, R tmin, bool behind_ok, R &best_t, int &best_i) {
    typedef double d4 __attribute__((ext_vector_type(4)));
    typedef const __attribute__((address_space(4))) d4 *cptr;
    const cptr p = (cptr)(exact12) + (size_t)i * 3;
    const d4 q0 = p[0], q2 = p[2];
    Prim4<R> s;
    s.cx = (R)q0.x; s.cy = (R)q0.y; s.cz = (R)q0.z;
    if (sizeof(R) == sizeof(double)) s.r2 = (R)q0.w;
    else { const R rad = (R)q2.z; s.r2 = rad * rad; }
    if (q2.y != 0.0) {
        const d4 q1 = p[1];
        const R t0 = (R)q1.w, t1 = (R)q2.x;
        const R f = (P.time - t0) / (t1 - t0), omf = R(1.0) - f;
        s.cx = (R)q0.x * omf + (R)q1.x * f; s.cy = (R)q0.y * omf + (R)q1.y * f; s.cz = (R)q0.z * omf + (R)q1.z * f;
    }
    R bq, cq, disc;
    sphere_test(s, P, coef<R>(a), bq, cq, disc);
    if (disc >= R(0)) sphere_roots<R>(bq, cq, disc, a, tmin, behind_ok, best_t, best_i, idx);
}

__device__ inline void cull_test_group(const CullGroup &G, int g, int last, const double *exact12, const Path<double> &P, const CullRay &c,
                                       double a, double tmin, bool behind_ok, double &best_t, int &best_i) {
    const float d0 = cull_disc(G, 0, c), d1 = cull_disc(G, 1, c), d2 = cull_disc(G, 2, c), d3 = cull_disc(G, 3, c);
    if (fmaxf(fmaxf(d0, d1), fmaxf(d2, d3)) >= 0.0f) {
        if (d0 >= 0.0f) exact_prim_test<double>(exact12, g, min(g, last), P, a, tmin, behind_ok, best_t, best_i);
        if (d1 >= 0.0f) exact_prim_test<double>(exact12, g + 1, min(g + 1, last), P, a, tmin, behind_ok, best_t, best_i);
        if (d2 >= 0.0f) exact_prim_test<double>(exact12, g + 2, min(g + 2, last), P, a, tmin, behind_ok, best_t, best_i);
        if (d3 >= 0.0f) exact_prim_test<double>(exact12, g + 3, min(g + 3, last), P, a, tmin, behind_ok, best_t, best_i);
    }
}

__device__ inline void scan_all_cull(SceneRef sc, const Path<double> &P, double a, double tmin, double &best_t, int &best_i) {
    const int n = sc.n_all;
    if (n <= 0) return;
    const int last = n - 1;
    const bool behind_ok = tmin >= 0.0;
    const float *cull20 = sc.cull20;
    const double *exact12 = sc.exact12;
    const CullRay c = make_cull_ray(P, a, sc.cull_t_lo, sc.cull_t_hi);
    CullGroup A = load_cull_group(cull20, 0);
    for (int g = 0; g < n; g += 8) {
        const CullGroup B = load_cull_group(cull20, (g >> 2) + 1);
        cull_test_group(A, g, last, exact12, P, c, a, tmin, behind_ok, best_t, best_i);
        A = load_cull_group(cull20, (g >> 2) + 2);
        cull_test_group(B, g + 4, last, exact12, P, c, a, tmin, behind_ok, best_t, best_i);
    }
}

#ifndef RTMI_EXIT_IBALLOT
#define RTMI_EXIT_IBALLOT 1
#endif
#ifndef RTMI_GRID_CHUNK
#define RTMI_GRID_CHUNK 1
#endif
#define RTMI_BVH_EMPTY ((int)0x80000000)
#ifndef RTMI_BVH_STACK
#define RTMI_BVH_STACK 32
#endif
#ifndef RTMI_TRACE_BLOCK
#define RTMI_TRACE_BLOCK 256
#endif
#define RTMI_BVH_STRIDE RTMI_TRACE_BLOCK

template <typename R, typename A>
__device__ inline void sphere_roots_any_order(R bq, R cq, R disc, const A &a, R tmin, bool behind_ok, R &best_t, int &best_i, int idx) {
    if (behind_ok && bq > R(0) && cq > R(0)) return;
    const R sq = Real<R>::sqrt_(disc);
    R t = quot<R>(-bq - sq, a);
    if (!(t > tmin)) t = quot<R>(-bq + sq, a);
    if ((t > tmin) && ((t < best_t) || (t == best_t && idx < best_i))) { best_t = t; best_i = idx; }
}

template <typename R, typename A>
__device__ inline void exact_prim_test_lane(const double *exact12, int code, const Path<R> &P, const A &a, R tmin, bool behind_ok, R &best_t, int &best_i) {
    const int bits = ~code;
    const int idx = bits & 0x3fffffff;
    const double2 *g = reinterpret_cast<const double2 *>(exact12 + (size_t)idx * 12);
    const double2 g0 = g[0], g1 = g[1];
    Prim4<R> s;
    s.cx = (R)g0.x; s.cy = (R)g0.y; s.cz = (R)g1.x;
    if (sizeof(R) == sizeof(double)) s.r2 = (R)g1.y;
    else { const R rad = (R)g[5].x; s.r2 = rad * rad; }
    if (bits & 0x40000000) {
        const double2 g2 = g[2], g3 = g[3], g4 = g[4];
        const R t0 = (R)g3.y, t1 = (R)g4.x;
        const R f = (P.time - t0) / (t1 - t0), omf = R(1.0) - f;
        s.cx = (R)g0.x * omf + (R)g2.x * f; s.cy = (R)g0.y * omf + (R)g2.y * f; s.cz = (R)g1.x * omf + (R)g3.x * f;
    }
    R bq, cq, disc;
    sphere_test(s, P, coef<R>(a), bq, cq, disc);
    if (disc >= R(0)) sphere_roots_any_order<R>(bq, cq, disc, a, tmin, behind_ok, best_t, best_i, idx);
}

typedef float v2f __attribute__((ext_vector_type(2)));
struct BvhRay { v2f ixy, izz, clxy, chxy, czz; float tmin_lo; bool ok, far, time_ok;
                unsigned shx, shy, shz; float cex, cey, cez, cxx, cxy, cxz; };
struct __attribute__((aligned(16))) Node16 { _Float16 p[12]; int cl, cr; };
__device__ inline bool slab_hit6(float ax, float bx, float ay, float by, float az, float bz, const float tmin_lo, const float best_hi, float &tnear) {
    const float tn = fmaxf(fmaxf(fminf(ax, bx), fminf(ay, by)), fmaxf(fminf(az, bz), tmin_lo));
    const float tf = fminf(fminf(fmaxf(ax, bx), fmaxf(ay, by)), fminf(fmaxf(az, bz), best_hi));
    tnear = tn;
// ... 175 lines not shown
        const float gmax = (float)(G - 1);
        const float ax = sc.grid_inv_x, az = sc.grid_inv_z, bx = -sc.grid_lo_x * ax, bz = -sc.grid_lo_z * az, ex = e * ax, ez = e * az;
        const float sx = fmaf(p0x, ax, bx), sz = fmaf(p0z, az, bz);
        int i0, i1, j0, j1, wi, wj;
        auto rect = [&]() {
            const float qx = fmaf(p1x, ax, bx), qz = fmaf(p1z, az, bz);
            const float fx0 = fminf(sx, qx) - ex, fx1 = fmaxf(sx, qx) + ex, fz0 = fminf(sz, qz) - ez, fz1 = fmaxf(sz, qz) + ez;
            i0 = (int)__builtin_amdgcn_fmed3f(floorf(fx0), 0.0f, gmax); i1 = (int)__builtin_amdgcn_fmed3f(floorf(fx1), 0.0f, gmax);
            j0 = (int)__builtin_amdgcn_fmed3f(floorf(fz0), 0.0f, gmax); j1 = (int)__builtin_amdgcn_fmed3f(floorf(fz1), 0.0f, gmax);
            wi = i1 - i0; wj = j1 - j0;
            return wi <= 1 && wj <= 1 && (wi + 1) * (wj + 1) <= sc.grid_kmax;
        };
        if (!rect()) {
#if RTMI_GRID_CHUNK
            const float gx = dx * ax, gz = dz * az;
            const float lx = gx >= 0.0f ? __builtin_amdgcn_fmed3f(floorf(sx - ex), 0.0f, gmax) + (2.0f - 1.0f / 256.0f) - ex : __builtin_amdgcn_fmed3f(floorf(sx + ex), 0.0f, gmax) - (1.0f - 1.0f / 256.0f) + ex;
            const float lz = gz >= 0.0f ? __builtin_amdgcn_fmed3f(floorf(sz - ez), 0.0f, gmax) + (2.0f - 1.0f / 256.0f) - ez : __builtin_amdgcn_fmed3f(floorf(sz + ez), 0.0f, gmax) - (1.0f - 1.0f / 256.0f) + ez;
            const float ts = tn + fminf((lx - sx) * __builtin_amdgcn_rcpf(gx), (lz - sz) * __builtin_amdgcn_rcpf(gz));
            p1x = fmaf(ts, dx, ox); p1z = fmaf(ts, dz, oz);
            if (!(ts > tn && ts < tf && sc.grid_walk && rect())) return kNoSplit;
            t_split = ts;
#else
            return kNoSplit;
#endif
        }
        node = sc.grid_cells[((wi + 2 * wj) * G + j0) * G + i0];
    } else if (!(tn > tf)) return kNoSplit;
    if (tall != RTMI_BVH_EMPTY) {
        if (node != RTMI_BVH_EMPTY) { *top = tos; top += stride; tos = node; }
        node = tall;
    }
    cur.node = node; cur.tos = tos; cur.top = top;
    return t_split;
}

template <bool COUNT = false, bool SLICE = false, typename Leaf, typename BestHi>
__device__ inline void bvh_traverse(SceneRef sc, const BvhRay &r, BvhCursor &cur, int min_lanes, Leaf leaf, BestHi best, unsigned *cnt = nullptr) {
    if (sc.bvh_node16) bvh_traverse_fmt<true, COUNT, SLICE>(sc, r, cur, min_lanes, leaf, best, cnt);
    else bvh_traverse_fmt<false, COUNT, SLICE>(sc, r, cur, min_lanes, leaf, best, cnt);
}

#define RTMI_BVH_SUSPEND_WORDS 6
template <typename R> __device__ inline void best_to_words(R t, int &w0, int &w1);
template <> __device__ inline void best_to_words<double>(double t, int &w0, int &w1) { w0 = __double2loint(t); w1 = __double2hiint(t); }
template <> __device__ inline void best_to_words<float>(float t, int &w0, int &w1) { w0 = __float_as_int(t); w1 = 0; }
template <typename R> __device__ inline R best_from_words(int w0, int w1);
template <> __device__ inline double best_from_words<double>(int w0, int w1) { return __hiloint2double(w1, w0); }
template <> __device__ inline float best_from_words<float>(int w0, int) { return __int_as_float(w0); }

template <typename R, bool COUNT = false, bool SLICE = false, bool CHUNK = true, typename Flat>
__device__ inline bool scan_bvh(SceneRef sc, int *stack, const Path<R> &P, R a, R tmin, R &best_t, int &best_i, Flat flat, unsigned *cnt = nullptr,
                                int *susp = nullptr, bool resume = false, int min_lanes = 0) {
    constexpr bool WALK = CHUNK && RTMI_GRID_CHUNK;
    const bool behind_ok = tmin >= R(0);
    const double *exact12 = sc.exact12;
    const BvhRay r = make_bvh_ray<R>(sc, P, a, tmin);
    constexpr int stride = RTMI_BVH_STRIDE;
    int *sw = susp + threadIdx.x;
    BvhCursor cur;
    float t_split = __builtin_inff(), t_from = -__builtin_inff();
    bool reenter = false;
    if (SLICE && resume) {
        cur.node = sw[0]; cur.tos = sw[stride];
        const int top_off = sw[2 * stride];
        cur.top = reinterpret_cast<int *>(reinterpret_cast<char *>(stack) + top_off);
        best_t = best_from_words<R>(sw[3 * stride], sw[4 * stride]);
        best_i = sw[5 * stride];
        if (WALK) {
            t_split = __int_as_float(stack[threadIdx.x]);
            if (top_off < 0) { reenter = true; t_from = t_split; t_split = __builtin_inff(); cur = bvh_cursor_at_root(sc, stack); }
        }
    } else {
        if (!r.ok) {
            if (COUNT) cnt[1] += (unsigned)sc.n_all;
            flat();
            return true;
        }
        cur = bvh_cursor_at_root(sc, stack);
    }
    const Quot<R> qa = make_quot<R>(a, tmin, best_t);
    RTMI_PH(PH_BVH_SETUP)
    if (!(SLICE && resume)) {
        if (COUNT) cnt[1] += (unsigned)sc.n_big;
        for (int k = 0; k < sc.n_big; ++k) exact_prim_test<R>(exact12, sc.big_idx[k], sc.big_idx[k], P, qa, tmin, behind_ok, best_t, best_i);
        RTMI_PH(PH_BIG)
    }
    auto leaf = [&](int code) { exact_prim_test_lane<R>(exact12, code, P, qa, tmin, behind_ok, best_t, best_i); };
    auto best = [&]() { return float_above((double)best_t); };
    const float e_rel = sizeof(R) == sizeof(float) ? 4.0e-3f + 1.0f / 65536.0f : 1.0f / 65536.0f;
    bool enter = CHUNK && sc.grid_n && (!(SLICE && resume) || reenter), first = !reenter;
    for (;;) {
        if (enter)
        {
            t_split = bvh_grid_entry(sc, r, (float)P.ox, (float)P.oy, (float)P.oz, (float)P.dx, (float)P.dy, (float)P.dz, best(), e_rel, cur, t_from, first);
            RTMI_PH(PH_GRID)
        }
        bvh_traverse<COUNT, SLICE>(sc, r, cur, min_lanes, leaf, best, cnt);
        if (SLICE && cur.node != RTMI_BVH_EMPTY) {
            int w0, w1;
            best_to_words<R>(best_t, w0, w1);
            sw[0] = cur.node; sw[stride] = cur.tos;
            sw[2 * stride] = (int)(reinterpret_cast<char *>(cur.top) - reinterpret_cast<char *>(stack));
            sw[3 * stride] = w0; sw[4 * stride] = w1; sw[5 * stride] = best_i;
            if (WALK) stack[threadIdx.x] = __float_as_int(t_split);
            return false;
        }
        if (!WALK) break;
        if (!(best_t > (R)t_split)) break;
        if (SLICE) {
            int w0, w1;
            best_to_words<R>(best_t, w0, w1);
            sw[0] = RTMI_BVH_EMPTY; sw[stride] = RTMI_BVH_EMPTY; sw[2 * stride] = -1;
            sw[3 * stride] = w0; sw[4 * stride] = w1; sw[5 * stride] = best_i;
            stack[threadIdx.x] = __float_as_int(t_split);
            return false;
        }
        cur = bvh_cursor_at_root(sc, stack);
        t_from = t_split; first = false; enter = true;
    }
    if (!r.time_ok)
        for (int k = 0; k < sc.n_moving_all; ++k) exact_prim_test_lane<R>(exact12, ~(sc.moving_all[k] | 0x40000000), P, qa, tmin, behind_ok, best_t, best_i);
    return true;
}

struct ExtHit { double t; int F, W; __device__ inline bool any() const { return F != 0x7fffffff; } };
__device__ inline int ext_winner(const ExtHit &H) { return H.any() ? max(H.F, H.W) : -1; }
__device__ inline void ext_update(ExtHit &H, double t, int idx, bool incl, bool ok = true) {
    const bool clt = t < H.t, ceq = t == H.t;
    const bool any = H.any();
    const bool take = ok & (clt | (incl & ceq & !any));
    const bool tie = ok & ceq & any;
    H.F = take ? idx : H.F;
    H.W = take ? (incl ? idx : -1) : H.W;
    H.t = take ? t : H.t;
    if (__builtin_expect(__any(tie), 0)) {
        H.F = tie ? min(H.F, idx) : H.F;
        if (incl) H.W = tie ? max(H.W, idx) : H.W;
    }
}

struct LocalRay { double ox, oy, oz, dx, dy, dz; };
template <bool UNIFORM> __device__ inline double ext_ld(const double *p, size_t i) {
    if (UNIFORM) return reinterpret_cast<const __attribute__((address_space(4))) double *>((const __attribute__((address_space(4))) void *)(p))[i];
    return p[i];
}
template <bool UNIFORM> __device__ inline int4 ext_ld_info(const int *p, int idx) {
    if (UNIFORM) {
        typedef int i4 __attribute__((ext_vector_type(4)));
        const i4 v = reinterpret_cast<const __attribute__((address_space(4))) i4 *>((const __attribute__((address_space(4))) void *)(p))[idx];
        return make_int4(v.x, v.y, v.z, v.w);
    }
    return reinterpret_cast<const int4 *>(p)[idx];
}
template <bool UNIFORM = false>
__device__ inline LocalRay ext_local_ray(SceneRef sc, int first, int count, const Path<double> &P) {
    LocalRay r = {P.ox, P.oy, P.oz, P.dx, P.dy, P.dz};
    for (int k = 0; k < count; ++k) {
        const size_t q = (size_t)(first + k) * 4;
        const double q0 = ext_ld<UNIFORM>(sc.ext_xf, q), q1 = ext_ld<UNIFORM>(sc.ext_xf, q + 1), q2 = ext_ld<UNIFORM>(sc.ext_xf, q + 2);
        if (q0 == 0.0) { const double q3 = ext_ld<UNIFORM>(sc.ext_xf, q + 3); r.ox = r.ox - q1; r.oy = r.oy - q2; r.oz = r.oz - q3; }
        else {
            const double sn = q1, cs = q2;
            const double ox = cs * r.ox - sn * r.oz, oz = sn * r.ox + cs * r.oz;
            const double dx = cs * r.dx - sn * r.dz, dz = sn * r.dx + cs * r.dz;
            r.ox = ox; r.oz = oz; r.dx = dx; r.dz = dz;
        }
    }
// ... 379 lines not shown
        cur.node = sw[0]; cur.tos = sw[stride];
        cur.top = reinterpret_cast<int *>(reinterpret_cast<char *>(stack) + sw[2 * stride]);
        H.t = __hiloint2double(sw[4 * stride], sw[3 * stride]);
        H.F = sw[5 * stride]; H.W = sw[6 * stride];
    } else {
        if (!r.ok) { if (COUNT) cnt[1] += (unsigned)sc.n_all; scan_all_cull_ext(sc, P, a, tmin, H, lo, hi); return true; }
        RTMI_PH(PH_BVH_SETUP)
        if (COUNT) cnt[1] += (unsigned)sc.n_big;
        for (int k = 0; k < sc.n_big; ++k) if (sc.big_idx[k] >= lo && sc.big_idx[k] < hi) ext_prim_test<true>(sc, sc.big_idx[k], P, tmin, H);
        cur = bvh_cursor_at_root(sc, stack);
        if (sc.n_mloc > 0 && !sc.media_seq && lo == 0 && H.t < 1e30) {
            const float ox = (float)P.ox, oy = (float)P.oy, oz = (float)P.oz, tb = (float)H.t;
            const float px = fmaf(tb, (float)P.dx, ox), py = fmaf(tb, (float)P.dy, oy), pz = fmaf(tb, (float)P.dz, oz);
            const float e = (fmaxf(fmaxf(fabsf(ox), fabsf(oy)), fabsf(oz)) + fmaxf(fmaxf(fabsf(px), fabsf(py)), fabsf(pz))) * (1.0f / 65536.0f);
            for (int k = 0; k < sc.n_mloc; ++k) {
                const float lx = sc.mloc_box[k][0] + e, ly = sc.mloc_box[k][1] + e, lz = sc.mloc_box[k][2] + e, hx = sc.mloc_box[k][3] - e, hy = sc.mloc_box[k][4] - e, hz = sc.mloc_box[k][5] - e;
                const bool in = ox >= lx && ox <= hx && oy >= ly && oy <= hy && oz >= lz && oz <= hz && px >= lx && px <= hx && py >= ly && py <= hy && pz >= lz && pz <= hz;
                if (in) cur.node = sc.mloc_root[k];
            }
        }
        RTMI_PH(PH_BIG)
    }
    auto leaf = [&](int code) {
        const int bits = ~code, idx = bits & 0x1fffffff;
        if (idx >= lo && idx < hi) {
            if (COUNT && (bits & RTMI_LEAF_BOX)) cnt[1] += 5;
#if RTMI_LEAF_RECORDS
            ext_leaf_test(sc, idx, (bits & RTMI_LEAF_BOX) != 0, P, tmin, H);
#else
            if (bits & RTMI_LEAF_BOX) ext_box_test<false>(sc, idx, P, tmin, H);
            else ext_prim_test<false>(sc, idx, P, tmin, H);
#endif
        }
    };
    auto best = [&]() { return ext_best_hi(H); };
    bvh_traverse<COUNT, SLICE>(sc, r, cur, min_lanes, leaf, best, cnt);
    if (SLICE && cur.node != RTMI_BVH_EMPTY) {
        sw[0] = cur.node; sw[stride] = cur.tos;
        sw[2 * stride] = (int)(reinterpret_cast<char *>(cur.top) - reinterpret_cast<char *>(stack));
        sw[3 * stride] = __double2loint(H.t); sw[4 * stride] = __double2hiint(H.t);
        sw[5 * stride] = H.F; sw[6 * stride] = H.W;
        return false;
    }
    if (!r.time_ok) {
        if (COUNT) cnt[1] += (unsigned)sc.n_moving_all;
        for (int k = 0; k < sc.n_moving_all; ++k) if (sc.moving_all[k] >= lo && sc.moving_all[k] < hi) ext_prim_test<true>(sc, sc.moving_all[k], P, tmin, H);
    }
    return true;
}

template <typename R>
__device__ inline void scan_moving(SceneRef sc, const Path<R> &P, R a, R tmin, R &best_t, int &best_i, int &best_orig) {
    const R a2 = R(2.0) * a, a4 = R(4.0) * a;
    for (int m = 0; m < sc.n_moving; ++m) {
        const double *g = sc.mov_geom + (size_t)m * RTMI_PRIM_STRIDE;
        const R t0 = (R)g[7], t1 = (R)g[8];
        const R f = (P.time - t0) / (t1 - t0), omf = R(1.0) - f;
        const R cx = (R)g[0] * omf + (R)g[4] * f, cy = (R)g[1] * omf + (R)g[5] * f, cz = (R)g[2] * omf + (R)g[6] * f;
        const R rad = (R)g[3];
        const R ocx = P.ox - cx, ocy = P.oy - cy, ocz = P.oz - cz;
        const R b = R(2.0) * dot3(ocx, ocy, ocz, P.dx, P.dy, P.dz);
        const R c = dot3(ocx, ocy, ocz, ocx, ocy, ocz) - rad * rad;
        const R disc = b * b - a4 * c;
        if (disc >= R(0)) {
            const R sq = Real<R>::sqrt_(disc);
            const int orig = sc.mov_orig[m];
            R t = (-b - sq) / a2;
            bool ok = (t > tmin) && ((t < best_t) || (t == best_t && orig < best_orig));
            if (!ok) {
                t = (-b + sq) / a2;
                ok = (t > tmin) && ((t < best_t) || (t == best_t && orig < best_orig));
            }
            if (ok) { best_t = t; best_i = sc.n_static + m; best_orig = orig; }
        }
    }
}

struct SegLog { double *rec; int max_seg; int n; };

template <typename R> struct HitRec { R t, px, py, pz, nx, ny, nz, u, v; int orig, kind, mat; };

#define RTMI_TEX_CHECKER2 100
#define RTMI_TEX_GRADIENT_REC 101
struct __attribute__((aligned(16))) MatRec { int mat_kind, tex, tex_kind, pad; double param, r, g, b; double scale, c1r, c1g, c1b; double inv_ri, r0; };

#define RTMI_PRIM_NEEDS_U 32
#define RTMI_PRIM_NEEDS_V 64
#define RTMI_PRIM_NEEDS_UV (RTMI_PRIM_NEEDS_U | RTMI_PRIM_NEEDS_V)
template <typename R> __device__ inline void resolve_hit(SceneRef sc, const Path<R> &P, R t, int orig, HitRec<R> &h, bool all_uv = true) {
    const double *g = sc.exact12 + (size_t)orig * 12;
    R cx = (R)g[0], cy = (R)g[1], cz = (R)g[2];
    h.orig = orig;
    const int2 km = reinterpret_cast<const int2 *>(sc.prim_km)[orig];
    if ((km.x & 15) == RTMI_PRIM_MOVING) {
        const R t0 = (R)g[7], t1 = (R)g[8];
        const R f = (P.time - t0) / (t1 - t0), omf = R(1.0) - f;
        cx = (R)g[0] * omf + (R)g[4] * f; cy = (R)g[1] * omf + (R)g[5] * f; cz = (R)g[2] * omf + (R)g[6] * f;
    }
    const int kind_flags = km.x;
    h.kind = kind_flags & 15;
    h.mat = km.y;
    h.t = t;
    h.px = P.dx * t + P.ox; h.py = P.dy * t + P.oy; h.pz = P.dz * t + P.oz;
    R nx = h.px - cx, ny = h.py - cy, nz = h.pz - cz;
    const R len = Real<R>::sqrt_(dot3(nx, ny, nz, nx, ny, nz));
    if (len > R(0)) { const R inv = R(1.0) / len; nx = nx * inv; ny = ny * inv; nz = nz * inv; }
    h.nx = nx; h.ny = ny; h.nz = nz;
    h.u = R(0); h.v = R(0);
    RTMI_PH(PH_HITREC)
    if (h.kind == RTMI_PRIM_UVSPHERE && (all_uv || (kind_flags & RTMI_PRIM_NEEDS_UV))) {
        h.u = h.v = R(0.5);
        if (all_uv || (kind_flags & RTMI_PRIM_NEEDS_U)) h.u = Real<R>::sphere_u(nx, nz);
        if (all_uv || (kind_flags & RTMI_PRIM_NEEDS_V)) h.v = Real<R>::sphere_v(ny);
        RTMI_PH(PH_UV)
    }
}

__device__ inline void leaf_xform_back(int xk, double a, double b, double c, double &px, double &py, double &pz, double &nx, double &nz) {
    if (xk == 1) { px = px + a; py = py + b; pz = pz + c; }
    else if (xk == 2) {
        const double rx = b * px + a * pz, rz = (-(a * px)) + b * pz;
        const double mx = b * nx + a * nz, mz = (-(a * nx)) + b * nz;
        px = rx; pz = rz; nx = mx; nz = mz;
    }
}
__device__ inline void resolve_hit_ext(SceneRef sc, const Path<double> &P, double t, int orig, HitRec<double> &h, bool all_uv = true) {
#if RTMI_LEAF_RECORDS
    {
        const double2 *q = reinterpret_cast<const double2 *>(sc.leaf_rec + (size_t)orig * RTMI_LEAF_REC_DOUBLES);
        const int4 hdr = *reinterpret_cast<const int4 *>(q);
        if (!hdr.y) {
            const double2 q1 = q[1], q2 = q[2], q3 = q[3], q4 = q[4], q5 = q[5], q6 = q[6];
            const int kind = hdr.x & 0xff;
            h.orig = orig; h.kind = kind; h.mat = sc.prim_mat[orig]; h.t = t;
            const bool want_uv = all_uv || (sc.prim_kind[orig] & RTMI_PRIM_NEEDS_UV);
            LocalRay r = {P.ox, P.oy, P.oz, P.dx, P.dy, P.dz};
            if (hdr.z | hdr.w) {
                leaf_xform(hdr.z, q3.y, q4.x, q4.y, r);
                leaf_xform(hdr.w, q5.x, q5.y, q6.x, r);
            }
            double px = r.dx * t + r.ox, py = r.dy * t + r.oy, pz = r.dz * t + r.oz;
            double nx, ny, nz;
            h.u = 0.0; h.v = 0.0;
            if (kind <= RTMI_PRIM_UVSPHERE) {
                nx = px - q1.x; ny = py - q1.y; nz = pz - q2.x;
                const double len = rt_sqrt(dot3(nx, ny, nz, nx, ny, nz));
                if (len > 0.0) { const double inv = 1.0 / len; nx = nx * inv; ny = ny * inv; nz = nz * inv; }
                if (kind == RTMI_PRIM_UVSPHERE && want_uv) Real<double>::sphere_uv(nx, ny, nz, &h.u, &h.v);
            } else {
                int ax, ua, va;
                rect_axes(kind, ax, ua, va);
                if (want_uv) {
                    const double x = pick3(ua, r.ox, r.oy, r.oz) + t * pick3(ua, r.dx, r.dy, r.dz), y = pick3(va, r.ox, r.oy, r.oz) + t * pick3(va, r.dx, r.dy, r.dz);
                    h.u = (x - q1.x) / (q2.x - q1.x); h.v = (y - q1.y) / (q2.y - q1.y);
                }
                nx = ax == 0 ? 1.0 : 0.0; ny = ax == 1 ? 1.0 : 0.0; nz = ax == 2 ? 1.0 : 0.0;
            }
            if (hdr.x & 0x100) { nx = -nx; ny = -ny; nz = -nz; }
            if (hdr.z | hdr.w) {
                leaf_xform_back(hdr.w, q5.x, q5.y, q6.x, px, py, pz, nx, nz);
                leaf_xform_back(hdr.z, q3.y, q4.x, q4.y, px, py, pz, nx, nz);
            }
            h.px = px; h.py = py; h.pz = pz; h.nx = nx; h.ny = ny; h.nz = nz;
            return;
        }
    }
#endif
    const int4 info = reinterpret_cast<const int4 *>(sc.ext_info)[orig];
    const LocalRay r = ext_local_ray(sc, info.z, info.w, P);
    const double *g = sc.exact12 + (size_t)orig * 12;
    const int kind = info.x;
    h.orig = orig; h.kind = kind; h.mat = sc.prim_mat[orig]; h.t = t;
    double px = r.dx * t + r.ox, py = r.dy * t + r.oy, pz = r.dz * t + r.oz;
    double nx, ny, nz;
    h.u = 0.0; h.v = 0.0;
    if (kind <= RTMI_PRIM_MOVING) {
        double cx = g[0], cy = g[1], cz = g[2];
        if (kind == RTMI_PRIM_MOVING) {
            const double t0 = g[7], t1 = g[8];
            const double f = (P.time - t0) / (t1 - t0), omf = 1.0 - f;
            cx = g[0] * omf + g[4] * f; cy = g[1] * omf + g[5] * f; cz = g[2] * omf + g[6] * f;
        }
        nx = px - cx; ny = py - cy; nz = pz - cz;
        const double len = rt_sqrt(dot3(nx, ny, nz, nx, ny, nz));
        if (len > 0.0) { const double inv = 1.0 / len; nx = nx * inv; ny = ny * inv; nz = nz * inv; }
        if (kind == RTMI_PRIM_UVSPHERE && (all_uv || (sc.prim_kind[orig] & RTMI_PRIM_NEEDS_UV))) {
            Real<double>::sphere_uv(nx, ny, nz, &h.u, &h.v);
        }
    } else if (kind == RTMI_PRIM_MEDIUM) {
        nx = 1.0; ny = 0.0; nz = 0.0;
    } else if (kind <= RTMI_PRIM_RECT_YZ) {
        int ax, ua, va;
        rect_axes(kind, ax, ua, va);
        if (all_uv || (sc.prim_kind[orig] & RTMI_PRIM_NEEDS_UV)) {
            const double x = pick3(ua, r.ox, r.oy, r.oz) + t * pick3(ua, r.dx, r.dy, r.dz), y = pick3(va, r.ox, r.oy, r.oz) + t * pick3(va, r.dx, r.dy, r.dz);
            h.u = (x - g[0]) / (g[2] - g[0]); h.v = (y - g[1]) / (g[3] - g[1]);
        }
        nx = ax == 0 ? 1.0 : 0.0; ny = ax == 1 ? 1.0 : 0.0; nz = ax == 2 ? 1.0 : 0.0;
    } else {
        if (all_uv || (sc.prim_kind[orig] & RTMI_PRIM_NEEDS_UV)) {
            double u = 0.0, v = 0.0, tt;
            tri_mt(g[0], g[1], g[2], g[3], g[4], g[5], g[6], g[7], g[8], r, u, v, tt);
            h.u = u; h.v = v;
        }
        cross3(g[3] - g[0], g[4] - g[1], g[5] - g[2], g[6] - g[0], g[7] - g[1], g[8] - g[2], nx, ny, nz);
    }
    if (info.y) { nx = -nx; ny = -ny; nz = -nz; }
    for (int k = info.w - 1; k >= 0; --k) {
        const double *q = sc.ext_xf + (size_t)(info.z + k) * 4;
        if (q[0] == 0.0) { px = px + q[1]; py = py + q[2]; pz = pz + q[3]; }
        else {
            const double sn = q[1], cs = q[2];
            const double rx = cs * px + sn * pz, rz = (-(sn * px)) + cs * pz;
            const double mx = cs * nx + sn * nz, mz = (-(sn * nx)) + cs * nz;
            px = rx; pz = rz; nx = mx; nz = mz;
        }
    }
    h.px = px; h.py = py; h.pz = pz; h.nx = nx; h.ny = ny; h.nz = nz;
}
template <typename R, bool EXT> __device__ inline void resolve_any(SceneRef sc, const Path<R> &P, R t, int orig, HitRec<R> &h, bool all_uv = true) { resolve_hit<R>(sc, P, t, orig, h, all_uv); }
template <> __device__ inline void resolve_any<double, true>(SceneRef sc, const Path<double> &P, double t, int orig, HitRec<double> &h, bool all_uv) { resolve_hit_ext(sc, P, t, orig, h, all_uv); }

template <typename R, bool F4 = false> __device__ inline bool scatter_emit(SceneRef sc, Path<R> &P, const HitRec<R> &h, R *att, R *emit, bool passenger = false) {
    const int mat = h.mat;
    const double2 *mq = reinterpret_cast<const double2 *>(sc.mat_rec + (size_t)mat * 12);
    const double2 m0 = mq[0], m1 = mq[1], m2 = mq[2];
    const int mk = (int)__double2loint(m0.x), mtex = (int)__double2hiint(m0.x), mtk = (int)__double2loint(m0.y);
    const R mparam = (R)m1.x;
    const R px = h.px, py = h.py, pz = h.pz, nx = h.nx, ny = h.ny, nz = h.nz;
    const bool is_light = !passenger && mk == RTMI_MAT_DIFFUSE_LIGHT;
    const bool live = !passenger && !is_light && P.depth > 0;
    const bool is_lamb = live && mk == RTMI_MAT_LAMBERTIAN, is_metal = live && mk == RTMI_MAT_METAL, is_diel = live && mk == RTMI_MAT_DIELECTRIC;
    const bool is_iso = F4 && live && mk == RTMI_MAT_ISOTROPIC;
    bool scat = false;
    emit[0] = emit[1] = emit[2] = R(0);
    R sdx = R(0), sdy = R(0), sdz = R(0);
    R atr = R(1), atg = R(1), atb = R(1);

    R dmag = R(0), ux = P.dx, uy = P.dy, uz = P.dz;
    if (is_metal || is_diel) {
        dmag = Real<R>::sqrt_(dot3(ux, uy, uz, ux, uy, uz));
        if (dmag > R(0)) { const R inv = R(1.0) / dmag; ux = ux * inv; uy = uy * inv; uz = uz * inv; }
        RTMI_PH(PH_DNORM)
    }
    R rx = R(0), ry = R(0), rz = R(0);
    RTMI_PH(PH_DIRS)
    rand_in_unit_sphere_wave(P, is_lamb || is_metal || is_iso, rx, ry, rz);
    RTMI_PH(PH_SAMPLER)
    if (is_lamb) {
        const R tx = (px + nx) + rx, ty = (py + ny) + ry, tz = (pz + nz) + rz;
        sdx = tx - px; sdy = ty - py; sdz = tz - pz;
        scat = true;
        RTMI_PH(PH_DIRS)
    } else if (is_iso) {
        sdx = rx; sdy = ry; sdz = rz;
        P.time = h.t;
        scat = true;
        RTMI_PH(PH_DIRS)
    } else if (is_metal) {
        const R fuzz = mparam;
        const R k = R(2.0) * dot3(ux, uy, uz, nx, ny, nz);
        const R rfx = ux - k * nx, rfy = uy - k * ny, rfz = uz - k * nz;
        sdx = rfx + fuzz * rx; sdy = rfy + fuzz * ry; sdz = rfz + fuzz * rz;
        scat = dot3(sdx, sdy, sdz, nx, ny, nz) > R(0);
        RTMI_PH(PH_DIRS)
    } else if (is_diel) {
        const R ri = mparam;
        const R dn = dot3(P.dx, P.dy, P.dz, nx, ny, nz);
        R onx, ony, onz, eta, cosine;
        if (dn > R(0)) { onx = -nx; ony = -ny; onz = -nz; eta = ri; cosine = ri * (dn / dmag); }
        else { onx = nx; ony = ny; onz = nz; eta = sizeof(R) == sizeof(double) ? (R)mq[5].x : R(1.0) / ri; cosine = -(dn / dmag); }
        const R dt = dot3(ux, uy, uz, onx, ony, onz);
        const R disc = R(1.0) - (eta * eta) * (R(1.0) - dt * dt);
        const R k = R(2.0) * dn;
        sdx = P.dx - k * nx; sdy = P.dy - k * ny; sdz = P.dz - k * nz;
        if (disc > R(0)) {
            R r0;
            if (sizeof(R) == sizeof(double)) r0 = (R)mq[5].y;
            else { r0 = (R(1.0) - ri) / (R(1.0) + ri); r0 = r0 * r0; }
            const R prob = r0 + (R(1.0) - r0) * pow5(R(1.0) - cosine);
            if (!(next_uniform(P) < prob)) {
                const R sq = Real<R>::sqrt_(disc);
                sdx = eta * (ux - onx * dt) - onx * sq;
                sdy = eta * (uy - ony * dt) - ony * sq;
                sdz = eta * (uz - onz * dt) - onz * sq;
            }
        }
        scat = true;
        RTMI_PH(PH_DIRS)
    }
    const bool want_tex = is_light || is_lamb || is_iso || (is_metal && scat);
    double turb = 0.0, turb_p0 = 0.0;
    bool turb_done = false;
    if (F4 && sizeof(R) == sizeof(double)) {
        const bool want_turb = want_tex && (mtk == RTMI_TEX_MARBLE || mtk == RTMI_TEX_PERLIN_TURB);
        const int n_turb = __popcll(__ballot(want_turb));
        if (n_turb > 0 && n_turb <= RTMI_TURB_WAVE_MAX) {
            double p1 = 0.0;
            if (want_turb) { const double *tp = sc.tex_param + (size_t)mtex * RTMI_TEX_STRIDE; turb_p0 = tp[0]; p1 = tp[1]; }
            const double s = mtk == RTMI_TEX_PERLIN_TURB ? turb_p0 : 1.0;
            turb = perlin_turbulence_wave(sc, want_turb, s * (double)px, s * (double)py, s * (double)pz, (int)p1);
            turb_done = want_turb;
        }
    }
    if (want_tex) {
        R tr, tg, tb;
        if (mtk == RTMI_TEX_CONSTANT) { tr = (R)m1.y; tg = (R)m2.x; tb = (R)m2.y; }
        else if (F4 && turb_done) {
            if (mtk == RTMI_TEX_PERLIN_TURB) tr = tg = tb = R(0.5) * ((R)turb + R(1.0));
            else tr = tg = tb = R(0.5) * (Real<R>::sin_((R)turb_p0 * pz + R(10.0) * (R)turb) + R(1.0));
        }
        else if (mtk == RTMI_TEX_CHECKER2) {
            const double2 m3 = mq[3], m4 = mq[4];
            const R scale = (R)m3.x;
            const int sx = sin_sign<R>(scale * px), sy = sin_sign<R>(scale * py), sz = sin_sign<R>(scale * pz);
            const bool neg = sx * sy * sz < 0;
            tr = neg ? (R)m1.y : (R)m3.y; tg = neg ? (R)m2.x : (R)m4.x; tb = neg ? (R)m2.y : (R)m4.y;
        } else if (mtk == RTMI_TEX_GRADIENT_REC) {
            const double2 *gq = reinterpret_cast<const double2 *>(sc.mat_grad + (size_t)mat * 12);
            const double2 g0 = gq[0], g1 = gq[1], g2 = gq[2], g3 = gq[3], g4 = gq[4], g5 = gq[5];
            const R u = h.u, v = h.v, omu = R(1.0) - u, omv = R(1.0) - v;
            const R a0 = (R)g1.y * omu + (R)g0.x * u, a1 = (R)g2.x * omu + (R)g0.y * u, a2 = (R)g2.y * omu + (R)g1.x * u;
            const R b0 = (R)g4.y * omu + (R)g3.x * u, b1 = (R)g5.x * omu + (R)g3.y * u, b2 = (R)g5.y * omu + (R)g4.x * u;
            tr = b0 * omv + a0 * v; tg = b1 * omv + a1 * v; tb = b2 * omv + a2 * v;
        } else tex_sample<R, F4>(sc, mtex, h.u, h.v, px, py, pz, tr, tg, tb);
        if (is_light) { emit[0] = R(0) + P.ar * tr; emit[1] = R(0) + P.ag * tg; emit[2] = R(0) + P.ab * tb; }
        else { atr = tr; atg = tg; atb = tb; }
        RTMI_PH(PH_TEXTURE)
    }
    if (!scat) return false;
    if (att) { att[0] = atr; att[1] = atg; att[2] = atb; }
    P.ox = px; P.oy = py; P.oz = pz; P.dx = sdx; P.dy = sdy; P.dz = sdz;
    P.ar = P.ar * atr; P.ag = P.ag * atg; P.ab = P.ab * atb;
    P.depth -= 1;
    return true;
}

template <typename R, bool EXT = false>
__device__ inline bool shade_segment(SceneRef sc, Path<R> &P, R t, int orig, SegLog *lg, R *emit, bool passenger = false) {
    emit[0] = emit[1] = emit[2] = R(0);
    if (!passenger && orig < 0) return false;
    HitRec<R> h;
    h.px = h.py = h.pz = h.nx = h.ny = h.nz = h.u = h.v = h.t = R(0); h.mat = 0; h.orig = 0; h.kind = 0;
    if (!passenger) {
        resolve_any<R, EXT>(sc, P, t, orig, h, false);
        RTMI_PH(PH_HITREC)
    }
    const bool scat = scatter_emit<R, EXT>(sc, P, h, nullptr, emit, passenger);
    if (lg && lg->n < lg->max_seg) {
        double *q = lg->rec + (size_t)lg->n * RTMI_SEG_REC;
        q[0] = h.orig; q[1] = h.t; q[2] = h.px; q[3] = h.py; q[4] = h.pz; q[5] = h.nx; q[6] = h.ny; q[7] = h.nz;
        q[8] = scat ? P.dx : 0; q[9] = scat ? P.dy : 0; q[10] = scat ? P.dz : 0; q[11] = scat ? 1.0 : 0.0;
        lg->n++;
    }
    return scat;
}

}
```

raytrace_clj_amd/csrc/scene_build.h:

```cpp
#pragma once
#include <unistd.h>

namespace {

struct BuildKnobs {
    int sah_levels = 1 << 20;
    int sweep_max = 0;
    double min_frac = 0.0;
    bool grid_off = false;
    int grid_side = 0;
    int grid_kmax = 4;
    bool grid_walk = true;
    bool mloc = false;
    int node16 = -1;
    bool box_leaf = false;
    bool small_scan = true;
    bool debug = false;
};
inline BuildKnobs read_build_knobs() {
    BuildKnobs k;
    if (const char *e = std::getenv("RTMI_BVH_SAH_LEVELS")) k.sah_levels = std::atoi(e);
    if (const char *e = std::getenv("RTMI_BVH_SWEEP_MAX")) k.sweep_max = std::atoi(e);
    if (const char *e = std::getenv("RTMI_BVH_MIN_FRAC")) k.min_frac = std::atof(e);
    if (const char *e = std::getenv("RTMI_GRID")) { k.grid_off = e[0] == '0'; k.grid_side = std::atoi(e); }
// ... 502 lines not shown
                    if (e32[0] >= 0 && std::isfinite(e32[0] + e32[1] + e32[2])) {
                        a32 += e32[0] * e32[1] + e32[1] * e32[2] + e32[2] * e32[0];
                        a16 += std::isfinite(e16[0] + e16[1] + e16[2]) ? e16[0] * e16[1] + e16[1] * e16[2] + e16[2] * e16[0] : INFINITY;
                    }
                }
                int c[2];
                std::memcpy(c, &q[12], 8);
                for (int k = 0; k < 2; ++k) if (c[k] >= 0 && c[k] != RTMI_BVH_EMPTY) c[k] /= 2;
                std::memcpy(reinterpret_cast<char *>(&out[n * 8]), h, 24);
                std::memcpy(reinterpret_cast<char *>(&out[n * 8]) + 24, c, 8);
            }
            part32[nb / 2048] = a32; part16[nb / 2048] = a16;
        });
        for (size_t k = 0; k < part32.size(); ++k) { area32 += part32[k]; area16 += part16[k]; }
        const bool use16 = K.node16 >= 0 ? K.node16 == 1 : (area16 <= 1.25 * area32);
        if (use16) {
            d.bvh_node16 = 1;
            d.bvh_root = d.bvh_root >= 0 ? d.bvh_root / 2 : d.bvh_root;
            for (int &c : grid_cells) if (c >= 0) c /= 2;
            for (int k = 0; k < d.n_mloc; ++k) if (d.mloc_root[k] >= 0) d.mloc_root[k] /= 2;
            if (d.grid_tall >= 0) d.grid_tall /= 2;
            return out;
        }
    }
    return B.nodes;
}

struct SceneArrays {
    int n_prims; const int32_t *prim_kind; const double *prim_geom; const int32_t *prim_mat;
    int n_mats; const int32_t *mat_kind; const int32_t *mat_tex; const double *mat_param;
    int n_tex; const int32_t *tex_kind; const double *tex_param; const int32_t *tex_child;
    int cam_kind; const double *cam; const int32_t *prim_flip; const int32_t *prim_xform;
    int n_xforms; const int32_t *xform_kind; const double *xform_param;
};

struct PackedScene {
    DevScene d{};
    std::vector<double> stat_geom, stat4_d, exact12, ext_xf, leaf_rec, mov_geom, mat_rec, mat_grad, mat_param, tex_param;
    std::vector<float> stat4_f, bvh_nodes, cull20;
    std::vector<int> stat_orig, grid_cells, moving_all, ext_info, mov_orig, prim_kind, prim_km, prim_mat, mat_kind, mat_tex, tex_kind, tex_child;
    std::vector<int> host_kind;
    std::map<int, std::array<double, 5>> media_fast_of;
    int bvh_node_count = 0, bvh_depth = 0, max_image = -1;
    bool uses_perlin = false;
    double t_tree0 = 0.0, t_tree1 = 0.0;
};

template <typename T> void pad_last(std::vector<T> &v, size_t rec) {
    const size_t n = v.size() / rec;
    if (n == 0) return;
    const std::vector<T> last(v.end() - (long)rec, v.end());
    while (v.size() < ((n + 7) / 8 * 8 + 8) * rec) v.insert(v.end(), last.begin(), last.end());
}

std::vector<char> texture_uv_use(const SceneArrays &a) {
    std::vector<char> uses((size_t)std::max(a.n_tex, 1), 0);
    bool changed = true;
    for (int pass = 0; pass <= a.n_tex && changed; ++pass) {
        changed = false;
        for (int t = 0; t < a.n_tex; ++t) {
            const int k = a.tex_kind[t];
            char u = k == RTMI_TEX_IMAGE ? 3 : 0;
            if (k == RTMI_TEX_UVGRADIENT) {
                const double *tp = a.tex_param + (size_t)t * RTMI_TEX_STRIDE;
                bool var_u = false, var_v = false;
                auto same = [&](int x, int y) { return std::memcmp(&tp[x], &tp[y], sizeof(double)) == 0; };
                for (int c = 0; c < 3; ++c) {
                    var_u = var_u || !same(c, 3 + c) || !same(6 + c, 9 + c);
                    var_v = var_v || !same(c, 6 + c) || !same(3 + c, 9 + c);
                }
                u = (char)((var_u ? 1 : 0) | (var_v ? 2 : 0));
            }
            if (k == RTMI_TEX_CHECKER || k == RTMI_TEX_FLIP_U || k == RTMI_TEX_FLIP_V)
                for (int c = 0; c < (k == RTMI_TEX_CHECKER ? 2 : 1); ++c) {
                    const int ch = a.tex_child[2 * (size_t)t + c];
                    if (ch >= 0 && ch < a.n_tex) u |= uses[(size_t)ch];
                }
            if (uses[(size_t)t] != u) { uses[(size_t)t] = u; changed = true; }
        }
    }
    return uses;
}

PackedScene pack_scene(const SceneArrays &a, const BuildKnobs &K) {
    PackedScene P;
    DevScene &d = P.d;
    std::memset(&d, 0, sizeof d);
    const int n_prims = a.n_prims;
    const double *cam = a.cam;
    bool has_ext = false;
    int n_world = 0, n_media = 0, media[16];
    for (int t = 0; t < a.n_tex; ++t) {
        if (a.tex_kind[t] > RTMI_TEX_CHECKER) has_ext = true;
        if (a.tex_kind[t] >= RTMI_TEX_PERLIN_NOISE && a.tex_kind[t] <= RTMI_TEX_MARBLE) P.uses_perlin = true;
        if (a.tex_kind[t] == RTMI_TEX_IMAGE) P.max_image = std::max(P.max_image, (int)a.tex_param[(size_t)t * RTMI_TEX_STRIDE]);
    }
    d.n_tex = a.n_tex; d.cam_kind = a.cam_kind;
    std::memcpy(d.cam, cam, 24 * sizeof(double));
    {
        bool fixed = a.cam_kind == RTMI_CAM_PINHOLE || cam[21] == 0.0;
        for (int k = 0; k < 3; ++k) fixed = fixed && !(cam[k] == 0.0 && std::signbit(cam[k])) && std::isfinite(cam[k]);
        for (int k = 12; k < 18; ++k) fixed = fixed && std::isfinite(cam[k]);
        d.cam_fixed_origin = fixed ? 1 : 0;
    }
    for (int k = 0; k < a.n_xforms; ++k) {
        const double *p = a.xform_param + (size_t)k * 3;
        const double rec[4] = {a.xform_kind[k] == RTMI_XFORM_TRANSLATE ? 0.0 : 1.0, p[0], p[1], p[2]};
        P.ext_xf.insert(P.ext_xf.end(), rec, rec + 4);
    }
    const double t_lo = a.cam_kind == RTMI_CAM_THINLENS ? std::min(cam[22], cam[23]) : 0.0;
    const double t_hi = a.cam_kind == RTMI_CAM_THINLENS ? std::max(cam[22], cam[23]) : 0.0;
    std::vector<float> cull;
    std::vector<BvhBox> wbox((size_t)n_prims);
    std::vector<char> bounded((size_t)n_prims, 0);
    std::vector<int> &pk = P.host_kind;
    pk.resize((size_t)n_prims);
    for (int i = 0; i < n_prims; ++i) {
        const double *g = a.prim_geom + (size_t)i * RTMI_PRIM_STRIDE;
        const int kind = a.prim_kind[i] & ~RTMI_PRIM_BOUNDARY;
        const bool is_boundary = (a.prim_kind[i] & RTMI_PRIM_BOUNDARY) != 0;
        const int xf_first = a.prim_xform ? a.prim_xform[2 * i] : 0, xf_count = a.prim_xform ? a.prim_xform[2 * i + 1] : 0;
        const int info[4] = {kind, a.prim_flip ? (a.prim_flip[i] & 1) : 0, xf_first, xf_count};
        P.ext_info.insert(P.ext_info.end(), info, info + 4);
        pk[(size_t)i] = kind;
        if (!is_boundary) n_world = i + 1;
        if (a.mat_kind[a.prim_mat[i]] == RTMI_MAT_ISOTROPIC) has_ext = true;
        if (kind == RTMI_PRIM_MEDIUM) {
            media[n_media++] = i;
            has_ext = true;
            P.exact12.insert(P.exact12.end(), {g[0], g[1], g[2], 0.0, 0.0, 0.0, 0.0, 0.0, 0.0, 0.0, 0.0, 0.0});
            cull.insert(cull.end(), {0.0f, 0.0f, 0.0f, 0.0f, 0.0f});
            continue;
        }
        const bool sphere_kernels = !is_boundary && kind <= RTMI_PRIM_MOVING && xf_count == 0 && !(a.prim_flip && a.prim_flip[i]);
        if (!sphere_kernels) has_ext = true;
        bounded[(size_t)i] = prim_world_box(kind, g, a.xform_kind, a.xform_param, xf_first, xf_count, t_lo, t_hi, wbox[(size_t)i]);
        const bool moving = kind == RTMI_PRIM_MOVING;
        const volatile double r2d = g[3] * g[3];
        if (sphere_kernels && moving) {
            P.mov_geom.insert(P.mov_geom.end(), g, g + RTMI_PRIM_STRIDE);
            P.mov_orig.push_back(i);
        } else if (sphere_kernels) {
            P.stat_geom.insert(P.stat_geom.end(), g, g + 4);
            P.stat_orig.push_back(i);
            const volatile float rf = (float)g[3];
            const volatile float r2f = rf * rf;
            P.stat4_d.insert(P.stat4_d.end(), {g[0], g[1], g[2], (double)r2d});
            P.stat4_f.insert(P.stat4_f.end(), {(float)g[0], (float)g[1], (float)g[2], (float)r2f});
        }
        if (kind > RTMI_PRIM_MOVING) P.exact12.insert(P.exact12.end(), {g[0], g[1], g[2], g[3], g[4], g[5], g[6], g[7], g[8], 0.0, 0.0, 0.0});
        else P.exact12.insert(P.exact12.end(), {g[0], g[1], g[2], (double)r2d, g[4], g[5], g[6], g[7], g[8], moving ? 1.0 : 0.0, g[3], 0.0});
        if (kind > RTMI_PRIM_MOVING || xf_count > 0) {
            float cf[3] = {0, 0, 0};
            double r2b = 3.0e38, w = 3.0e38;
            if (bounded[(size_t)i]) {
                const BvhBox &b = wbox[(size_t)i];
                double slack = 0.0, rb2 = 0.0, cn = 0.0;
                for (int k = 0; k < 3; ++k) {
                    const double cm = 0.5 * (b.lo[k] + b.hi[k]);
                    cf[k] = (float)cm;
                    slack += std::fabs(cm - (double)cf[k]);
                    rb2 += 0.25 * (b.hi[k] - b.lo[k]) * (b.hi[k] - b.lo[k]);
                    cn += std::fabs((double)cf[k]);
                }
                const double rb = (std::sqrt(rb2) + slack + 1e-4) * (1.0 + 1e-6);
                r2b = rb * rb * (1.0 + 1e-6);
// ... 35 lines not shown
    if (K.box_leaf)
    for (int i = 0; i + 5 < n_world; ++i) {
        static const int want[6] = {RTMI_PRIM_RECT_XY, RTMI_PRIM_RECT_XY, RTMI_PRIM_RECT_XZ, RTMI_PRIM_RECT_XZ, RTMI_PRIM_RECT_YZ, RTMI_PRIM_RECT_YZ};
        bool ok = true;
        for (int k = 0; k < 6 && ok; ++k) {
            ok = pk[(size_t)i + k] == want[k];
            if (a.prim_xform) ok = ok && a.prim_xform[2 * (i + k)] == a.prim_xform[2 * i] && a.prim_xform[2 * (i + k) + 1] == a.prim_xform[2 * i + 1];
        }
        if (!ok) continue;
        const double *q = a.prim_geom + (size_t)i * RTMI_PRIM_STRIDE;
        const double x0 = q[0], y0 = q[1], x1 = q[2], y1 = q[3], z1 = q[4], z0 = q[RTMI_PRIM_STRIDE + 4];
        const double expect[6][5] = {{x0, y0, x1, y1, z1}, {x0, y0, x1, y1, z0}, {x0, z0, x1, z1, y1}, {x0, z0, x1, z1, y0}, {y0, z0, y1, z1, x1}, {y0, z0, y1, z1, x0}};
        for (int k = 0; k < 6 && ok; ++k) for (int c = 0; c < 5; ++c) ok = ok && std::memcmp(&q[(size_t)k * RTMI_PRIM_STRIDE + c], &expect[k][c], sizeof(double)) == 0;
        if (!ok) continue;
        box_first[(size_t)i] = 1;
        P.exact12[(size_t)i * 12 + 5] = z0;
        i += 5;
    }
    pad_last(P.exact12, 12);
    pad_last(cull, 5);
    P.cull20.resize(cull.size() / 20 * 20);
    for (size_t g = 0; g < P.cull20.size(); g += 20)
        for (int k = 0; k < 4; ++k) for (int f = 0; f < 5; ++f) P.cull20[g + 4 * f + k] = cull[g + 5 * k + f];
    d.n_all = n_world; d.cull_t_lo = t_lo; d.cull_t_hi = t_hi;
    d.n_media = n_media;
    for (int k = 0; k < n_media; ++k) { d.media_idx[k] = media[k]; d.media_lo[k] = media[k]; }
    P.t_tree0 = now_ms();
    std::vector<BvhBox> media_boxes;
    for (int k = 0; k < n_media; ++k) {
        const double *mg = a.prim_geom + (size_t)media[k] * RTMI_PRIM_STRIDE;
        const int fb = (int)mg[1], nb = (int)mg[2];
        BvhBox u = box_empty();
        bool ok = true;
        for (int q = fb; q < fb + nb; ++q) { ok = ok && bounded[(size_t)q]; if (ok) box_grow(u, wbox[(size_t)q]); }
        if (ok) media_boxes.push_back(u);
    }
    P.bvh_nodes = build_bvh(d, n_world, pk.data(), wbox, bounded, cam, !has_ext, P.grid_cells, box_first, K, &P.bvh_depth, &media_boxes);
    P.bvh_node_count = (int)(P.bvh_nodes.size() / (d.bvh_node16 ? 8 : 16));
    if (K.debug)
        fprintf(stderr, "[rtmi] tree: %d node records of %d bytes (%.2f MB), depth %d, %d big primitives, %d box leaves; entry grid %d x %d cells, %zu rectangle trees\n", P.bvh_node_count,
                d.bvh_node16 ? 32 : 64, P.bvh_node_count * (d.bvh_node16 ? 32.0 : 64.0) / 1e6, P.bvh_depth, d.n_big, (int)std::count(box_first.begin(), box_first.end(), (char)1), d.grid_n, d.grid_n, P.grid_cells.size());
    if (K.debug && d.n_mloc) fprintf(stderr, "[rtmi] %d medium neighbourhood tree(s)\n", d.n_mloc);
    P.t_tree1 = now_ms();
    for (int i = 0; i < n_world; ++i) if (pk[(size_t)i] == RTMI_PRIM_MOVING) P.moving_all.push_back(i);
    d.n_moving_all = (int)P.moving_all.size();
    d.has_ext = has_ext ? 1 : 0;
    d.small_scan = (has_ext && n_world <= RTMI_SMALL_SCAN_MAX && K.small_scan) ? 1 : 0;
    P.leaf_rec.assign((size_t)std::max(n_prims, 1) * RTMI_LEAF_REC_DOUBLES, 0.0);
    for (int i = 0; i < n_prims; ++i) {
        double *q = &P.leaf_rec[(size_t)i * RTMI_LEAF_REC_DOUBLES];
        const int *info = &P.ext_info[(size_t)i * 4];
        const int kind = info[0], xf_first = info[2], xf_count = info[3];
        int hdr[4] = {kind | (info[1] ? 0x100 : 0), 0, 0, 0};
        const bool simple = (kind == RTMI_PRIM_SPHERE || kind == RTMI_PRIM_UVSPHERE || (kind >= RTMI_PRIM_RECT_XY && kind <= RTMI_PRIM_RECT_YZ)) && xf_count <= 2;
        if (!simple) hdr[1] = 1;
        else {
            for (int c = 0; c < 5; ++c) q[2 + c] = P.exact12[(size_t)i * 12 + c];
            for (int k = 0; k < xf_count; ++k) {
                const double *xp = a.xform_param + (size_t)(xf_first + k) * 3;
                hdr[2 + k] = a.xform_kind[xf_first + k] == RTMI_XFORM_TRANSLATE ? 1 : 2;
                q[7 + 3 * k] = xp[0]; q[8 + 3 * k] = xp[1]; q[9 + 3 * k] = xp[2];
            }
            if (box_first[(size_t)i]) q[13] = P.exact12[(size_t)i * 12 + 5];
        }
        std::memcpy(q, hdr, sizeof hdr);
    }
    P.ext_info.insert(P.ext_info.end(), {RTMI_PRIM_MEDIUM, 0, 0, 0});
    const std::vector<char> uses = texture_uv_use(a);
    P.prim_mat.assign(a.prim_mat, a.prim_mat + n_prims);
    P.prim_kind = pk;
    for (int i = 0; i < n_prims; ++i) {
        const int m = P.prim_mat[(size_t)i], t = (m >= 0 && m < a.n_mats) ? a.mat_tex[m] : -1;
        if (pk[(size_t)i] == RTMI_PRIM_UVSPHERE) {
            const int bits = (t < 0 || t >= a.n_tex) ? 3 : uses[(size_t)t];
            if (bits & 1) P.prim_kind[(size_t)i] |= RTMI_PRIM_NEEDS_U;
            if (bits & 2) P.prim_kind[(size_t)i] |= RTMI_PRIM_NEEDS_V;
        } else if (pk[(size_t)i] >= RTMI_PRIM_RECT_XY && pk[(size_t)i] <= RTMI_PRIM_TRIANGLE) {
            if (t < 0 || t >= a.n_tex || uses[(size_t)t]) P.prim_kind[(size_t)i] |= RTMI_PRIM_NEEDS_UV;
        }
    }
    P.prim_km.assign((size_t)std::max(n_prims, 1) * 2, 0);
    for (int i = 0; i < n_prims; ++i) { P.prim_km[2 * (size_t)i] = P.prim_kind[(size_t)i]; P.prim_km[2 * (size_t)i + 1] = P.prim_mat[(size_t)i]; }
    P.mat_rec.assign((size_t)std::max(a.n_mats, 1) * 12, 0.0);
    P.mat_grad.assign((size_t)std::max(a.n_mats, 1) * 12, 0.0);
    for (int m = 0; m < a.n_mats; ++m) {
        MatRec r;
        std::memset(&r, 0, sizeof(r));
        r.mat_kind = a.mat_kind[m]; r.tex = a.mat_tex[m]; r.param = a.mat_param[m];
        if (a.mat_kind[m] == RTMI_MAT_DIELECTRIC) {
            const volatile double ri = a.mat_param[m];
            const volatile double inv = 1.0 / ri, num = 1.0 - ri, den = 1.0 + ri;
            const volatile double q = num / den;
            const volatile double r0 = q * q;
            r.inv_ri = inv; r.r0 = r0;
        }
        r.tex_kind = (r.tex >= 0 && r.tex < a.n_tex) ? a.tex_kind[r.tex] : -1;
        if (r.tex_kind == RTMI_TEX_CONSTANT) { const double *tp = a.tex_param + (size_t)r.tex * RTMI_TEX_STRIDE; r.r = tp[0]; r.g = tp[1]; r.b = tp[2]; }
        if (r.tex_kind == RTMI_TEX_UVGRADIENT) {
            std::memcpy(&P.mat_grad[(size_t)m * 12], a.tex_param + (size_t)r.tex * RTMI_TEX_STRIDE, 12 * sizeof(double));
            r.tex_kind = RTMI_TEX_GRADIENT_REC;
        }
        if (r.tex_kind == RTMI_TEX_CHECKER) {
            const int c0 = a.tex_child[2 * (size_t)r.tex], c1 = a.tex_child[2 * (size_t)r.tex + 1];
            if (c0 >= 0 && c0 < a.n_tex && c1 >= 0 && c1 < a.n_tex && a.tex_kind[c0] == RTMI_TEX_CONSTANT && a.tex_kind[c1] == RTMI_TEX_CONSTANT) {
                const double *t0 = a.tex_param + (size_t)c0 * RTMI_TEX_STRIDE, *t1 = a.tex_param + (size_t)c1 * RTMI_TEX_STRIDE;
                r.tex_kind = RTMI_TEX_CHECKER2;
                r.scale = a.tex_param[(size_t)r.tex * RTMI_TEX_STRIDE];
                r.r = t0[0]; r.g = t0[1]; r.b = t0[2]; r.c1r = t1[0]; r.c1g = t1[1]; r.c1b = t1[2];
            }
        }
        static_assert(sizeof(MatRec) == 96, "MatRec is twelve doubles");
        std::memcpy(&P.mat_rec[(size_t)m * 12], &r, sizeof(r));
    }
    P.mat_kind.assign(a.mat_kind, a.mat_kind + a.n_mats); P.mat_tex.assign(a.mat_tex, a.mat_tex + a.n_mats); P.mat_param.assign(a.mat_param, a.mat_param + a.n_mats);
    P.tex_kind.assign(a.tex_kind, a.tex_kind + a.n_tex); P.tex_child.assign(a.tex_child, a.tex_child + 2 * (size_t)a.n_tex);
    P.tex_param.assign(a.tex_param, a.tex_param + (size_t)a.n_tex * RTMI_TEX_STRIDE);
    for (int k = 0; k < n_media; ++k) {
        const int m = media[k];
        const int fb = (int)a.prim_geom[(size_t)m * RTMI_PRIM_STRIDE + 1], nb = (int)a.prim_geom[(size_t)m * RTMI_PRIM_STRIDE + 2];
        if (nb != 1 || fb < 0 || fb >= n_prims) continue;
        if (pk[(size_t)fb] != RTMI_PRIM_SPHERE && pk[(size_t)fb] != RTMI_PRIM_UVSPHERE) continue;
        if (a.prim_xform && (a.prim_xform[2 * m + 1] != 0 || a.prim_xform[2 * fb + 1] != 0)) continue;
        const double *e = &P.exact12[0];
        P.media_fast_of[m] = {e[(size_t)m * 12], e[(size_t)fb * 12], e[(size_t)fb * 12 + 1], e[(size_t)fb * 12 + 2], e[(size_t)fb * 12 + 3]};
    }
    return P;
}

}
```

Baseline: 7741 Msamples/s.

## Replace divisions with reciprocal-Newton paths and fold u-invariant gradient textures

Several arithmetic shortcuts land together. Camera pixel coordinates use a precomputed reciprocal of nx and ny. Normal and direction normalisation use a hardware rcp refined by Newton steps, with a guard for out-of-range inputs. The dielectric cosine reuses one quotient. Big-sphere tests take only the far root when the whole wavefront is inside the sphere. Gradient textures whose two u-corners are equal are folded into a single v lerp. Each is meant to cut f64 divide or arithmetic cost in the hot path, at the price of extra guard branches and possible last-ulp differences. Probes are added to check exactness.

After: 7729 Msamples/s. No clear change (-0.2%).

```diff
diff --git a/include/rtmi.h b/include/rtmi.h
--- a/include/rtmi.h
+++ b/include/rtmi.h
@@ -126,6 +126,10 @@
 int rtmi_probe_math2(rtmi_ctx *ctx, int32_t n, const double *abc, double tmin, double tmax, int32_t n_slots, double *out);
 int rtmi_probe_math(rtmi_ctx *ctx, int32_t n, const double *abc, double tmin, double tmax, double *out);
 
+#define RTMI_PROBE_RECIP_SLOTS 5
+int rtmi_probe_recip(rtmi_ctx *ctx, int32_t n, const double *abc, double *out);
+int rtmi_test_fold_gradient(const double *corners, double *out_ab);
+
 int rtmi_test_build_tree(int32_t n, const double *geom, const double *cam, int32_t threads, uint64_t *out_hash, int32_t *out_info, double *out_ms);
 int rtmi_test_half_outward(double x, int32_t up);
 
diff --git a/raytrace_clj_amd/_ffi.py b/raytrace_clj_amd/_ffi.py
--- a/raytrace_clj_amd/_ffi.py
+++ b/raytrace_clj_amd/_ffi.py
@@ -16,7 +16,7 @@
     "rtmi_device_info", "rtmi_scene_create", "rtmi_scene_create_ex", "rtmi_scene_set_perlin", "rtmi_scene_set_images", "rtmi_scene_set_media_calls", "rtmi_scene_set_media_mode", "rtmi_scene_set_media_calls_narrowed", "rtmi_scene_device_bytes", "rtmi_scene_destroy", "rtmi_render", "rtmi_render_device",
     "rtmi_render_tiles_device", "rtmi_local_tiles", "rtmi_assemble_device", "rtmi_last_trace_ms", "rtmi_last_reduce_ms", "rtmi_probe_hit",
     "rtmi_probe_paths", "rtmi_probe_camera", "rtmi_probe_texture", "rtmi_probe_scatter", "rtmi_probe_rng",
-    "rtmi_sample_key", "rtmi_test_half_outward", "rtmi_test_build_tree", "rtmi_probe_arith", "rtmi_probe_math", "rtmi_probe_math2", "rtmi_last_traversal_counters",
+    "rtmi_sample_key", "rtmi_test_half_outward", "rtmi_test_build_tree", "rtmi_probe_arith", "rtmi_probe_math", "rtmi_probe_math2", "rtmi_probe_recip", "rtmi_test_fold_gradient", "rtmi_last_traversal_counters",
     "rtmi_scene_clone", "rtmi_render_multi", "rtmi_render_multi_device", "rtmi_last_gather_ms",
     "rtmi_last_gather_path", "rtmi_rccl_probe", "rtmi_stream_idle", "rtmi_last_passes", "rtmi_last_accel",
     "rtmi_render_progressive", "rtmi_render_progressive_device", "rtmi_progressive_samples", "rtmi_progressive_release",
@@ -85,6 +85,8 @@
     L.rtmi_test_half_outward.argtypes = [C.c_double, i32]
     L.rtmi_probe_math.argtypes = [vp, i32, vp, C.c_double, C.c_double, vp]
     L.rtmi_probe_math2.argtypes = [vp, i32, vp, C.c_double, C.c_double, i32, vp]
+    L.rtmi_probe_recip.argtypes = [vp, i32, vp, vp]
+    L.rtmi_test_fold_gradient.argtypes = [vp, vp]
     L.rtmi_last_traversal_counters.argtypes = [vp, C.POINTER(u64), C.POINTER(u64)]
     L.rtmi_scene_clone.argtypes = [vp, vp, C.POINTER(vp)]
     L.rtmi_render_multi.argtypes = [i32, C.POINTER(vp), i32, i32, i32, i32, u64, i32, vp, vp, vp]
diff --git a/raytrace_clj_amd/core.py b/raytrace_clj_amd/core.py
--- a/raytrace_clj_amd/core.py
+++ b/raytrace_clj_amd/core.py
@@ -244,6 +244,20 @@
     out = np.zeros((len(abc), slots))
     check(_ffi.lib().rtmi_probe_math2(ctx.handle, len(abc), ptr(abc), tmin, tmax, slots, ptr(out)))
     return out
+
+
+def probe_recip(abc, ctx=None):
+    ctx = ctx or default_context()
+    abc = np.ascontiguousarray(abc, np.float64).reshape(-1, 3)
+    out = np.zeros((len(abc), 5))
+    check(_ffi.lib().rtmi_probe_recip(ctx.handle, len(abc), ptr(abc), ptr(out)))
+    return out
+
+
+def fold_gradient(corners):
+    corners = np.ascontiguousarray(corners, np.float64).reshape(12)
+    out = np.zeros(6)
+    return out if _ffi.lib().rtmi_test_fold_gradient(ptr(corners), ptr(out)) == 1 else None
 
 
 def sample_key(seed, pixel, sample):
diff --git a/raytrace_clj_amd/csrc/rtmi.hip b/raytrace_clj_amd/csrc/rtmi.hip
--- a/raytrace_clj_amd/csrc/rtmi.hip
+++ b/raytrace_clj_amd/csrc/rtmi.hip
@@ -70,6 +70,7 @@
     u64 *trav;
     int susp_off;
     int stash_off;
+    double nx_d, ny_d, inv_nx, inv_ny;
 };
 #ifndef RTMI_QUEUE_BLOCK
 #define RTMI_QUEUE_BLOCK 256
@@ -230,10 +231,17 @@
     }
 }
 
+#ifndef RTMI_CAM_DIV_CONST
+#define RTMI_CAM_DIV_CONST 1
+#endif
+template <typename R> __device__ inline R pixel_coord(R x, int n, double, double) { return x / (R)n; }
+#if RTMI_CAM_DIV_CONST
+template <> __device__ inline double pixel_coord<double>(double x, int, double n_d, double rn) { return div_const(x, n_d, rn); }
+#endif
 template <typename R> __device__ inline void start_sample(SceneRef sc, const TraceParams &tp, int i, int j, int s, Path<R> &P) {
     seed_stream(P, sample_key(tp.seed, (u64)j * (u64)tp.nx + (u64)i, (u64)s), 0u);
-    const R u = ((R)(float)i + next_uniform(P)) / (R)tp.nx;
-    const R v = ((R)(float)j + next_uniform(P)) / (R)tp.ny;
+    const R u = pixel_coord<R>((R)(float)i + next_uniform(P), tp.nx, tp.nx_d, tp.inv_nx);
+    const R v = pixel_coord<R>((R)(float)j + next_uniform(P), tp.ny, tp.ny_d, tp.inv_ny);
     get_ray<R>(sc, u, v, P);
     P.ar = P.ag = P.ab = R(1);
     P.depth = tp.depth;
@@ -1113,6 +1121,7 @@
         const int s_count = std::min(s_per_pass, s_end - s_begin);
         TraceParams tp;
         tp.nx = nx; tp.ny = ny; tp.depth = depth; tp.seed = seed; tp.tiles_x = tiles_x_of(nx);
+        { const volatile double dnx = (double)nx, dny = (double)ny; tp.nx_d = dnx; tp.ny_d = dny; tp.inv_nx = 1.0 / dnx; tp.inv_ny = 1.0 / dny; }
         tp.n_local_tiles = n_local; tp.tile_ids = reinterpret_cast<const int *>(c->tile_ids.p);
         tp.s_begin = s_begin; tp.s_count = s_count; tp.samples = c->samples.p; tp.counters = cnt;
         tp.prims_per_tile = (c->scan_variant >= SCAN_SGPR || s->dev.has_ext) ? 0 : ppt; tp.n_ptiles = nptiles;
@@ -1225,7 +1234,7 @@
 RTMI_EXPORT int rtmi_test_half_outward(double x, int32_t up) { return (int)half_outward((float)x, up != 0); }
 RTMI_EXPORT const char *rtmi_last_error(void) { return g_err.c_str(); }
 RTMI_EXPORT const char *rtmi_backend_name(void) { return "hip-gfx950"; }
-RTMI_EXPORT int rtmi_version(void) { return 205; }
+RTMI_EXPORT int rtmi_version(void) { return 206; }
 RTMI_EXPORT uint64_t rtmi_sample_key(uint64_t seed, uint64_t pixel, uint64_t sample) { return sample_key(seed, pixel, sample); }
 
 RTMI_EXPORT int rtmi_init(int device, uint32_t flags, rtmi_ctx **out_ctx) {
@@ -2278,6 +2287,39 @@
     for (int j = 0; j < n_slots; ++j) out[(size_t)k * n_slots + j] = o[j];
 }
 
+__global__ void probe_recip_kernel(int n, const double *abc, double *out) {
+    const int k = blockIdx.x * blockDim.x + threadIdx.x;
+    if (k >= n) return;
+    const double a = abc[3 * k], b = abc[3 * k + 1], c = abc[3 * k + 2];
+    const Quot<double> q = make_recip<double>(b);
+    double *o = out + (size_t)k * RTMI_PROBE_RECIP_SLOTS;
+    o[0] = recip_one<double>(q);
+    o[1] = (double)(RTMI_RCP_UNSCALED && q.fast);
+    o[2] = recip_quot<double>(a, q);
+    o[3] = (double)(q.fast && recip_num_ok(a));
+    o[4] = pixel_coord<double>(a, (int)c, c, 1.0 / c);
+}
+
+RTMI_EXPORT int rtmi_probe_recip(rtmi_ctx *c, int32_t n, const double *abc, double *out) {
+    if (!ctx_ok(c)) return fail(RTMI_E_STATE, "invalid context handle");
+    if (n <= 0 || !abc || !out) return fail(RTMI_E_ARG, "bad arguments");
+    HIP_TRY(hipSetDevice(c->device));
+    Tmp tmp;
+    double *d_in = (double *)tmp.up(abc, (size_t)n * 3 * sizeof(double));
+    double *d_out = (double *)tmp.alloc((size_t)n * RTMI_PROBE_RECIP_SLOTS * sizeof(double));
+    if (!d_in || !d_out) return fail(RTMI_E_NOMEM, "probe buffers");
+    const unsigned grid = (unsigned)((n + kBlock - 1) / kBlock);
+    hipLaunchKernelGGL(probe_recip_kernel, dim3(grid), dim3(kBlock), 0, c->stream, n, d_in, d_out);
+    PROBE_EPILOGUE()
+    HIP_TRY(hipMemcpy(out, d_out, (size_t)n * RTMI_PROBE_RECIP_SLOTS * sizeof(double), hipMemcpyDeviceToHost));
+    return RTMI_OK;
+}
+
+RTMI_EXPORT int rtmi_test_fold_gradient(const double *corners, double *out_ab) {
+    if (!corners || !out_ab) return -1;
+    return fold_gradient(corners, out_ab) ? 1 : 0;
+}
+
 RTMI_EXPORT int rtmi_probe_arith(rtmi_ctx *c, int32_t n, const double *abc, double *out) {
     if (!ctx_ok(c)) return fail(RTMI_E_STATE, "invalid context handle");
     if (n <= 0 || !abc || !out) return fail(RTMI_E_ARG, "bad arguments");
diff --git a/raytrace_clj_amd/csrc/rtmi_device.h b/raytrace_clj_amd/csrc/rtmi_device.h
--- a/raytrace_clj_amd/csrc/rtmi_device.h
+++ b/raytrace_clj_amd/csrc/rtmi_device.h
@@ -237,6 +237,39 @@
     q.r = ::fma(r, ::fma(-a, r, 1.0), r);
     return q;
 }
+#ifndef RTMI_RCP_UNSCALED
+#define RTMI_RCP_UNSCALED 1
+#endif
+#ifndef RTMI_DIEL_ONE_QUOT
+#define RTMI_DIEL_ONE_QUOT 1
+#endif
+template <typename R> __device__ inline Quot<R> make_recip(R x) { return Quot<R>{x}; }
+template <> __device__ inline Quot<double> make_recip<double>(double x) {
+    Quot<double> q;
+    q.a = x;
+    q.fast = (unsigned)__double2hiint(x) - (823u << 20) < (400u << 20);
+    double r = __builtin_amdgcn_rcp(x);
+    r = ::fma(r, ::fma(-x, r, 1.0), r);
+    q.r = ::fma(r, ::fma(-x, r, 1.0), r);
+    return q;
+}
+template <typename R> __device__ inline R recip_one(const Quot<R> &q) { return R(1.0) / q.a; }
+template <> __device__ inline double recip_one<double>(const Quot<double> &q) {
+#if RTMI_RCP_UNSCALED
+    if (__builtin_expect(!q.fast, 0)) return 1.0 / q.a;
+    return ::fma(::fma(-q.a, q.r, 1.0), q.r, q.r);
+#else
+    return 1.0 / q.a;
+#endif
+}
+template <typename R> __device__ inline R recip_quot(R n, const Quot<R> &q) { return n / q.a; }
+__device__ inline bool recip_num_ok(double n) { return ((unsigned)__double2hiint(n) & 0x7fffffffu) - (223u << 20) < (1368u << 20); }
+template <> __device__ inline double recip_quot<double>(double n, const Quot<double> &q) {
+    if (__builtin_expect(!(q.fast && recip_num_ok(n)), 0)) return n / q.a;
+    const double t = n * q.r;
+    return ::fma(::fma(-q.a, t, n), q.r, t);
+}
+
 template <typename R> __device__ inline R quot(R n, R a) { return n / a; }
 template <typename R> __device__ inline R quot(R n, const Quot<R> &a) { return a(n); }
 template <typename R> __device__ inline R coef(R a) { return a; }
@@ -608,6 +641,14 @@
     }
     if (ok) { best_t = t; best_i = idx; }
 }
+#ifndef RTMI_INSIDE_FAR_ROOT
+#define RTMI_INSIDE_FAR_ROOT 1
+#endif
+template <typename R, typename A>
+__device__ inline void sphere_root_far(R bq, R disc, const A &a, R tmin, R &best_t, int &best_i, int idx) {
+    const R t = quot<R>(-bq + Real<R>::sqrt_(disc), a);
+    if ((t > tmin) && (t < best_t)) { best_t = t; best_i = idx; }
+}
 
 template <typename R> __device__ inline void sphere_test(const Prim4<R> &s, const Path<R> &P, R a, R &bq, R &cq, R &disc) {
     const R ocx = P.ox - s.cx, ocy = P.oy - s.cy, ocz = P.oz - s.cz;
@@ -715,7 +756,7 @@
     return fmaf(b, b, t2);
 }
 
-template <typename R, typename A>
+template <typename R, typename A, bool BIG = false>
 __device__ inline void exact_prim_test(const double *exact12, int i, int idx, const Path<R> &P, const A &a, R tmin, bool behind_ok, R &best_t, int &best_i) {
     typedef double d4 __attribute__((ext_vector_type(4)));
     typedef const __attribute__((address_space(4))) d4 *cptr;
@@ -733,7 +774,11 @@
     }
     R bq, cq, disc;
     sphere_test(s, P, coef<R>(a), bq, cq, disc);
-    if (disc >= R(0)) sphere_roots<R>(bq, cq, disc, a, tmin, behind_ok, best_t, best_i, idx);
+    if (disc >= R(0)) {
+        const R b_abs = bq < R(0) ? -bq : bq, b_min = sizeof(R) == sizeof(double) ? R(0x1p-500) : R(0x1p-60);
+        if (BIG && RTMI_INSIDE_FAR_ROOT && behind_ok && !__any(!((cq < R(0)) & (b_abs >= b_min)))) sphere_root_far<R>(bq, disc, a, tmin, best_t, best_i, idx);
+        else sphere_roots<R>(bq, cq, disc, a, tmin, behind_ok, best_t, best_i, idx);
+    }
 }
 
 __device__ inline void cull_test_group(const CullGroup &G, int g, int last, const double *exact12, const Path<double> &P, const CullRay &c,
@@ -1075,7 +1120,7 @@
     RTMI_PH(PH_BVH_SETUP)
     if (!(SLICE && resume)) {
         if (COUNT) cnt[1] += (unsigned)sc.n_big;
-        for (int k = 0; k < sc.n_big; ++k) exact_prim_test<R>(exact12, sc.big_idx[k], sc.big_idx[k], P, qa, tmin, behind_ok, best_t, best_i);
+        for (int k = 0; k < sc.n_big; ++k) exact_prim_test<R, Quot<R>, true>(exact12, sc.big_idx[k], sc.big_idx[k], P, qa, tmin, behind_ok, best_t, best_i);
         RTMI_PH(PH_BIG)
     }
     auto leaf = [&](int code) { exact_prim_test_lane<R>(exact12, code, P, qa, tmin, behind_ok, best_t, best_i); };
@@ -1621,6 +1666,11 @@
 
 #define RTMI_TEX_CHECKER2 100
 #define RTMI_TEX_GRADIENT_REC 101
+#define RTMI_TEX_GRADIENT_FOLD 102
+#define RTMI_MAT_GRAD_STRIDE 18
+#ifndef RTMI_GRADIENT_FOLD
+#define RTMI_GRADIENT_FOLD 1
+#endif
 struct __attribute__((aligned(16))) MatRec { int mat_kind, tex, tex_kind, pad; double param, r, g, b; double scale, c1r, c1g, c1b; double inv_ri, r0; };
 
 #define RTMI_PRIM_NEEDS_U 32
@@ -1643,7 +1693,7 @@
     h.px = P.dx * t + P.ox; h.py = P.dy * t + P.oy; h.pz = P.dz * t + P.oz;
     R nx = h.px - cx, ny = h.py - cy, nz = h.pz - cz;
     const R len = Real<R>::sqrt_(dot3(nx, ny, nz, nx, ny, nz));
-    if (len > R(0)) { const R inv = R(1.0) / len; nx = nx * inv; ny = ny * inv; nz = nz * inv; }
+    if (len > R(0)) { const R inv = recip_one<R>(make_recip<R>(len)); nx = nx * inv; ny = ny * inv; nz = nz * inv; }
     h.nx = nx; h.ny = ny; h.nz = nz;
     h.u = R(0); h.v = R(0);
     RTMI_PH(PH_HITREC)
@@ -1760,7 +1810,7 @@
 template <typename R, bool EXT> __device__ inline void resolve_any(SceneRef sc, const Path<R> &P, R t, int orig, HitRec<R> &h, bool all_uv = true) { resolve_hit<R>(sc, P, t, orig, h, all_uv); }
 template <> __device__ inline void resolve_any<double, true>(SceneRef sc, const Path<double> &P, double t, int orig, HitRec<double> &h, bool all_uv) { resolve_hit_ext(sc, P, t, orig, h, all_uv); }
 
-template <typename R, bool F4 = false> __device__ inline bool scatter_emit(SceneRef sc, Path<R> &P, const HitRec<R> &h, R *att, R *emit, bool passenger = false) {
+template <typename R, bool F4 = false> __device__ inline bool scatter_emit(SceneRef sc, Path<R> &P, const HitRec<R> &h, R *att, R *emit, bool passenger = false, bool hit_uv = false) {
     const int mat = h.mat;
     const double2 *mq = reinterpret_cast<const double2 *>(sc.mat_rec + (size_t)mat * 12);
     const double2 m0 = mq[0], m1 = mq[1], m2 = mq[2];
@@ -1776,10 +1826,14 @@
     R sdx = R(0), sdy = R(0), sdz = R(0);
     R atr = R(1), atg = R(1), atb = R(1);
 
-    R dmag = R(0), ux = P.dx, uy = P.dy, uz = P.dz;
+    R dmag = R(0), ux = P.dx, uy = P.dy, uz = P.dz, dn_q = R(0);
     if (is_metal || is_diel) {
         dmag = Real<R>::sqrt_(dot3(ux, uy, uz, ux, uy, uz));
-        if (dmag > R(0)) { const R inv = R(1.0) / dmag; ux = ux * inv; uy = uy * inv; uz = uz * inv; }
+        const Quot<R> rq = make_recip<R>(dmag);
+        if (dmag > R(0)) { const R inv = recip_one<R>(rq); ux = ux * inv; uy = uy * inv; uz = uz * inv; }
+#if RTMI_DIEL_ONE_QUOT
+        if (is_diel) dn_q = recip_quot<R>(dot3(P.dx, P.dy, P.dz, nx, ny, nz), rq);
+#endif
         RTMI_PH(PH_DNORM)
     }
     R rx = R(0), ry = R(0), rz = R(0);
@@ -1807,8 +1861,13 @@
         const R ri = mparam;
         const R dn = dot3(P.dx, P.dy, P.dz, nx, ny, nz);
         R onx, ony, onz, eta, cosine;
+#if RTMI_DIEL_ONE_QUOT
+        if (dn > R(0)) { onx = -nx; ony = -ny; onz = -nz; eta = ri; cosine = ri * dn_q; }
+        else { onx = nx; ony = ny; onz = nz; eta = sizeof(R) == sizeof(double) ? (R)mq[5].x : R(1.0) / ri; cosine = -dn_q; }
+#else
         if (dn > R(0)) { onx = -nx; ony = -ny; onz = -nz; eta = ri; cosine = ri * (dn / dmag); }
         else { onx = nx; ony = ny; onz = nz; eta = sizeof(R) == sizeof(double) ? (R)mq[5].x : R(1.0) / ri; cosine = -(dn / dmag); }
+#endif
         const R dt = dot3(ux, uy, uz, onx, ony, onz);
         const R disc = R(1.0) - (eta * eta) * (R(1.0) - dt * dt);
         const R k = R(2.0) * dn;
@@ -1855,8 +1914,13 @@
             const int sx = sin_sign<R>(scale * px), sy = sin_sign<R>(scale * py), sz = sin_sign<R>(scale * pz);
             const bool neg = sx * sy * sz < 0;
             tr = neg ? (R)m1.y : (R)m3.y; tg = neg ? (R)m2.x : (R)m4.x; tb = neg ? (R)m2.y : (R)m4.y;
-        } else if (mtk == RTMI_TEX_GRADIENT_REC) {
-            const double2 *gq = reinterpret_cast<const double2 *>(sc.mat_grad + (size_t)mat * 12);
+        } else if (RTMI_GRADIENT_FOLD && sizeof(R) == sizeof(double) && hit_uv && mtk == RTMI_TEX_GRADIENT_FOLD) {
+            const double2 *gq = reinterpret_cast<const double2 *>(sc.mat_grad + (size_t)mat * RTMI_MAT_GRAD_STRIDE + 12);
+            const double2 f0 = gq[0], f1 = gq[1], f2 = gq[2];
+            const R v = h.v, omv = R(1.0) - v;
+            tr = (R)f1.y * omv + (R)f0.x * v; tg = (R)f2.x * omv + (R)f0.y * v; tb = (R)f2.y * omv + (R)f1.x * v;
+        } else if (mtk == RTMI_TEX_GRADIENT_REC || mtk == RTMI_TEX_GRADIENT_FOLD) {
+            const double2 *gq = reinterpret_cast<const double2 *>(sc.mat_grad + (size_t)mat * RTMI_MAT_GRAD_STRIDE);
             const double2 g0 = gq[0], g1 = gq[1], g2 = gq[2], g3 = gq[3], g4 = gq[4], g5 = gq[5];
             const R u = h.u, v = h.v, omu = R(1.0) - u, omv = R(1.0) - v;
             const R a0 = (R)g1.y * omu + (R)g0.x * u, a1 = (R)g2.x * omu + (R)g0.y * u, a2 = (R)g2.y * omu + (R)g1.x * u;
@@ -1885,7 +1949,7 @@
         resolve_any<R, EXT>(sc, P, t, orig, h, false);
         RTMI_PH(PH_HITREC)
     }
-    const bool scat = scatter_emit<R, EXT>(sc, P, h, nullptr, emit, passenger);
+    const bool scat = scatter_emit<R, EXT>(sc, P, h, nullptr, emit, passenger, true);
     if (lg && lg->n < lg->max_seg) {
         double *q = lg->rec + (size_t)lg->n * RTMI_SEG_REC;
         q[0] = h.orig; q[1] = h.t; q[2] = h.px; q[3] = h.py; q[4] = h.pz; q[5] = h.nx; q[6] = h.ny; q[7] = h.nz;
diff --git a/raytrace_clj_amd/csrc/scene_build.h b/raytrace_clj_amd/csrc/scene_build.h
--- a/raytrace_clj_amd/csrc/scene_build.h
+++ b/raytrace_clj_amd/csrc/scene_build.h
@@ -608,6 +608,19 @@
     return uses;
 }
 
+inline bool fold_gradient(const double *tp, double *out) {
+    for (int c = 0; c < 3; ++c)
+        if (std::memcmp(&tp[c], &tp[3 + c], sizeof(double)) != 0 || std::memcmp(&tp[6 + c], &tp[9 + c], sizeof(double)) != 0) return false;
+    const volatile double u = 0.5;
+    const volatile double omu = 1.0 - u;
+    for (int c = 0; c < 3; ++c) {
+        const volatile double a_l = tp[3 + c] * omu, a_r = tp[c] * u, b_l = tp[9 + c] * omu, b_r = tp[6 + c] * u;
+        const volatile double a = a_l + a_r, b = b_l + b_r;
+        out[c] = a; out[3 + c] = b;
+    }
+    return true;
+}
+
 PackedScene pack_scene(const SceneArrays &a, const BuildKnobs &K) {
     PackedScene P;
     DevScene &d = P.d;
@@ -809,7 +822,13 @@
     P.prim_km.assign((size_t)std::max(n_prims, 1) * 2, 0);
     for (int i = 0; i < n_prims; ++i) { P.prim_km[2 * (size_t)i] = P.prim_kind[(size_t)i]; P.prim_km[2 * (size_t)i + 1] = P.prim_mat[(size_t)i]; }
     P.mat_rec.assign((size_t)std::max(a.n_mats, 1) * 12, 0.0);
-    P.mat_grad.assign((size_t)std::max(a.n_mats, 1) * 12, 0.0);
+    P.mat_grad.assign((size_t)std::max(a.n_mats, 1) * RTMI_MAT_GRAD_STRIDE, 0.0);
+    std::vector<char> half_u((size_t)std::max(a.n_mats, 1), (char)(has_ext ? 0 : 1));
+    for (int i = 0; i < n_prims; ++i) {
+        const int m = P.prim_mat[(size_t)i];
+        if (m < 0 || m >= a.n_mats) continue;
+        if ((P.prim_kind[(size_t)i] & (15 | RTMI_PRIM_NEEDS_UV)) != (RTMI_PRIM_UVSPHERE | RTMI_PRIM_NEEDS_V)) half_u[(size_t)m] = 0;
+    }
     for (int m = 0; m < a.n_mats; ++m) {
         MatRec r;
         std::memset(&r, 0, sizeof(r));
@@ -824,8 +843,10 @@
         r.tex_kind = (r.tex >= 0 && r.tex < a.n_tex) ? a.tex_kind[r.tex] : -1;
         if (r.tex_kind == RTMI_TEX_CONSTANT) { const double *tp = a.tex_param + (size_t)r.tex * RTMI_TEX_STRIDE; r.r = tp[0]; r.g = tp[1]; r.b = tp[2]; }
         if (r.tex_kind == RTMI_TEX_UVGRADIENT) {
-            std::memcpy(&P.mat_grad[(size_t)m * 12], a.tex_param + (size_t)r.tex * RTMI_TEX_STRIDE, 12 * sizeof(double));
+            double *gr = &P.mat_grad[(size_t)m * RTMI_MAT_GRAD_STRIDE];
+            std::memcpy(gr, a.tex_param + (size_t)r.tex * RTMI_TEX_STRIDE, 12 * sizeof(double));
             r.tex_kind = RTMI_TEX_GRADIENT_REC;
+            if (RTMI_GRADIENT_FOLD && half_u[(size_t)m] && fold_gradient(gr, gr + 12)) r.tex_kind = RTMI_TEX_GRADIENT_FOLD;
         }
         if (r.tex_kind == RTMI_TEX_CHECKER) {
             const int c0 = a.tex_child[2 * (size_t)r.tex], c1 = a.tex_child[2 * (size_t)r.tex + 1];
```
